# rasd3/TODA

Hardware: NVIDIA B200
Metric: frames/s voxelize+VoxelResBackBone8x fwd+bwd (higher is better)
Workload: dtype bf16

## Files before the change

### include/toda_b200.h

```cpp
#ifndef TODA_B200_H
#define TODA_B200_H

#include <stddef.h>
#include <stdint.h>

#ifdef __cplusplus
extern "C" {
#endif

#define TODA_OK 0
#define TODA_ERR_INVALID (-1)
#define TODA_ERR_CUDA (-2)
#define TODA_ERR_WORKSPACE (-3)
#define TODA_ERR_UNSUPPORTED (-4)

#define TODA_ORDER_FIRST_APPEARANCE 0
#define TODA_ORDER_CANONICAL 1

const char *toda_last_error(void);
int toda_version(void);
long long toda_launch_count(void);
int toda_device_info(int *sm_count_host, int *cc_major_host, int *cc_minor_host);

size_t toda_index_bytes(int batch, int D, int H, int W);
int toda_index_insert(void *index, int batch, int D, int H, int W, const int32_t *coords, int n, void *stream);
int toda_index_insert_strided(void *index_out, int batch, int oD, int oH, int oW, const int32_t *in_coords, int n_in,
                              const int *ksize_host, const int *stride_host, const int *pad_host, void *stream);
int toda_index_build(void *index, int batch, int D, int H, int W, int32_t *out_coords, int cap, int32_t *n_out,
                     void *stream);
int toda_index_rows(const void *index, int batch, int D, int H, int W, const int32_t *coords, int n, int32_t *rows,
                    void *stream);
int toda_index_release(void *index, int batch, int D, int H, int W, const int32_t *coords, int n, void *stream);

#define TODA_SELECT_RANGE_XY 0
#define TODA_SELECT_RECT_XY 1
#define TODA_SELECT_SECTOR 2
#define TODA_SELECT_BOXES 3
size_t toda_points_select_workspace_bytes(int n);
int toda_points_select(const float *points, int n, int stride, int x_col, const int32_t *frame_offsets, int batch, int mode,
                       const double *params_host, int invert, int add_batch_col, float *out, int32_t *out_offsets,
                       void *workspace, size_t workspace_bytes, void *stream);

#define TODA_WORLD_FLIP_X 0
#define TODA_WORLD_FLIP_Y 1
#define TODA_WORLD_ROTATE 2
#define TODA_WORLD_SCALE 3
int toda_points_world_transform(const float *points, int n, int stride, int x_col, const int32_t *frame_offsets, int batch,
                                int n_steps, const int *kinds_host, const float *params_host, float *out, void *stream);

size_t toda_voxelize_workspace_bytes(int64_t n_points, int batch, const int *grid_host, int max_points,
                                     int max_voxels);
int toda_voxelize_hard(const float *points, int64_t n_points, int point_stride, int xyz_col, int feat_col,
                       int num_features, const int32_t *frame_offsets, int batch, const float *range_host,
                       const float *vsize_host, const int *grid_host, int max_points, int max_voxels, int order,
                       float *voxels, int32_t *coords, int32_t *num_points, int32_t *voxel_counts, void *workspace,
                       size_t workspace_bytes, void *stream);

int toda_mean_vfe_fwd(const float *voxels, const void *num_points, int num_is_float, int n_voxels, int max_points,
                      int num_features, float *voxel_features, void *stream);
int toda_mean_vfe_bwd(const float *d_voxel_features, const void *num_points, int num_is_float, int n_voxels,
                      int max_points, int num_features, float *d_voxels, void *stream);

int toda_rulebook_subm(const void *index, int batch, int D, int H, int W, const int32_t *coords, int n,
                       const int *ksize_host, int32_t *nbr, void *stream);
int toda_rulebook_sparse(const void *index_in, int iD, int iH, int iW, const void *index_out, int oD, int oH, int oW,
                         int batch, const int32_t *in_coords, int n_in, const int32_t *out_coords, int n_out,
                         const int *ksize_host, const int *stride_host, const int *pad_host, int32_t *nbr_fwd,
                         int32_t *nbr_bwd, void *stream);

size_t toda_parity_order_workspace_bytes(int n);
int toda_parity_order(const int32_t *coords, int n, const int *stride_host, const int *pad_host, int32_t *order,
                      int32_t *pos_of_row, void *workspace, size_t workspace_bytes, void *stream);

#define TODA_CONV_FP32 0
#define TODA_CONV_BF16 1
#define TODA_CONV_BF16X3 2
int toda_weight_repack(const float *w_param, int kvol, int cin, int cout, int transpose, int mirror_k, float *w_out,
                       void *stream);
size_t toda_spconv_fwd_workspace_bytes(int n_in, int cin, int cout, int kvol, int precision);
int toda_table_tile_masks(const int32_t *nbr, int n_out, int kvol, uint32_t *masks, void *stream);
int toda_spconv_uses_tensor_cores(int cin, int cout, int kvol, int precision);
int toda_spconv_wgrad_uses_tensor_cores(int cin, int cout, int kvol, int precision);
int toda_spconv_fwd(const float *x, const void *x_bf16, int n_in, int cin, const int32_t *nbr, int n_out, int kvol,
                    const float *w, int cout, const float *bias, float *y, const int32_t *out_rows,
                    const uint32_t *tile_masks, double *bn_sums, int precision, void *workspace, size_t workspace_bytes,
                    void *stream);
int toda_tile_plan_capacity(int channels);
int toda_table_tile_plan(const int32_t *nbr, int n_out, int kvol, int ngroups, int cap, uint16_t *lidx, int32_t *rows,
                         int32_t *cnt, void *stream);
int toda_spconv_fwd_plan(const float *x, const void *x_bf16, int n_in, int cin, const int32_t *nbr, int n_out, int kvol,
                         const float *w, int cout, const float *bias, const float *addend, float *y,
                         const int32_t *out_rows, const uint32_t *tile_masks, const uint16_t *plan_lidx,
                         const int32_t *plan_rows, const int32_t *plan_cnt, int plan_groups, int plan_cap, double *bn_sums,
                         const void *w_bf16, int precision, void *workspace, size_t workspace_bytes, void *stream);
int toda_weight_kmajor_bf16(const float *w, int kvol, int cin, int cout, void *w_bf16, void *stream);
size_t toda_spconv_wgrad_workspace_bytes(int n_in, int n_out, int kvol, int cin, int cout, int precision);
int toda_spconv_wgrad(const float *x, const void *x_bf16, int n_in, int cin, const int32_t *nbr, int n_out, int kvol,
                      const uint32_t *tile_masks, const float *dy, const void *dy_bf16, int cout, float *dw_param,
                      void *workspace, size_t workspace_bytes, int precision, void *stream);
int toda_spconv_wgrad_row_splits(const uint32_t *tile_masks, int n_out, int kvol, int cin, int cout, int *groups,
                                 int *splits, int32_t *row_begin, void *stream);

size_t toda_bn_workspace_bytes(int channels);
int toda_bn_local_sums(const float *y, const double *epilogue_sums, int n, int channels, double *sums, double *count,
                       void *workspace, size_t workspace_bytes, void *stream);
int toda_bn_eval_coeffs(const float *gamma, const float *beta, const float *running_mean, const float *running_var,
                        float eps, int channels, float *scale, float *shift, void *stream);
int toda_bn_apply(const float *y, int n, int channels, const float *scale, const float *shift, const float *residual,
                  int relu, float *a, void *a_bf16, void *stream);
int toda_bn_apply_sums(const float *y, int n, int channels, const double *sums, const double *count, const float *gamma,
                       const float *beta, float eps, float momentum, float *running_mean, float *running_var, float *scale,
                       float *shift, float *save_mean, float *save_rstd, const float *residual, int relu, float *a,
                       void *a_bf16, void *stream);
int toda_bn_bwd_reduce(const float *da, const float *a, const float *y, int n, int channels, const float *save_mean,
                       const float *save_rstd, int relu, double *red, float *dgamma, float *dbeta, void *workspace,
                       size_t workspace_bytes, void *stream);
int toda_bn_bwd_finish(const float *da, const float *a, const float *y, int n, int channels, const float *gamma,
                       const float *save_mean, const float *save_rstd, int relu, int training, const double *red,
                       const double *count, float *dy, void *dy_bf16, float *dresidual, float *dbias, void *workspace,
                       size_t workspace_bytes, void *stream);
int toda_bn_bwd(const float *da, const float *a, const float *y, int n, int channels, const float *gamma,
                const float *save_mean, const float *save_rstd, int relu, int training, float *dy, void *dy_bf16,
                float *dresidual, float *dgamma, float *dbeta, float *dbias, void *workspace, size_t workspace_bytes,
                void *stream);
int toda_col_sum(const float *dy, int n, int channels, float *out, void *workspace, size_t workspace_bytes,
                 void *stream);

typedef struct {
    const float *x; const void *x_bf16; int n_in, cin; const int32_t *nbr; int n_out, kvol;
    const float *w; const void *w_bf16 ; int cout; const float *bias ;
    const uint32_t *tile_masks ;
    const uint16_t *plan_lidx ; const int32_t *plan_rows; const int32_t *plan_cnt; int plan_groups, plan_cap;
    int precision; void *conv_ws; size_t conv_ws_bytes;
    const float *gamma; const float *beta; float eps, momentum; float *running_mean; float *running_var; int training;
    const float *residual ; int relu;
    float *y; double *sums; float *stats; float *a; void *a_bf16 ;
    void *bn_ws; size_t bn_ws_bytes;
} toda_layer_fwd_args;
typedef struct {
    const float *da; const float *a_mask; const float *y; int n_out, cout; const float *gamma; const float *mean; const float *rstd;
    int relu, training; float *dy; void *dy_bf16 ; float *dres ; float *dgamma; float *dbeta;
    void *bn_ws; size_t bn_ws_bytes;
    const float *x; const void *x_bf16 ; int n_in, cin, kvol;
    int need_dx; const int32_t *dgrad_nbr; const float *wt; const void *wt_bf16 ;
    const int32_t *dgrad_out_rows ; const uint32_t *dgrad_masks ;
    const uint16_t *dplan_lidx ; const int32_t *dplan_rows; const int32_t *dplan_cnt; int dplan_groups, dplan_cap;
    const float *addend ; float *dx;
    int need_dw; const int32_t *nbr_fwd; const uint32_t *fwd_masks ; float *dw;
    void *wgrad_ws; size_t wgrad_ws_bytes;
    int need_db; float *db;
    int precision; void *conv_ws; size_t conv_ws_bytes;
} toda_layer_bwd_args;
int toda_layer_fwd(const toda_layer_fwd_args *args, void *stream);
int toda_layer_bwd(const toda_layer_bwd_args *args, void *stream);
int toda_layer_fwd_stats(const toda_layer_fwd_args *args, double *local_sums, void *stream);
int toda_layer_fwd_apply(const toda_layer_fwd_args *args, const double *global_sums, void *stream);
int toda_layer_bwd_reduce(const toda_layer_bwd_args *args, double *local_red, void *stream);
int toda_layer_bwd_finish(const toda_layer_bwd_args *args, const double *global_red, const double *global_count, void *stream);

int toda_bev_scatter_fwd(const float *features, const int32_t *coords, int n, int channels, int batch, int D, int H,
                         int W, float *out, void *stream);
int toda_bev_scatter_bwd(const float *d_out, const int32_t *coords, int n, int channels, int batch, int D, int H,
                         int W, float *d_features, void *stream);

int toda_gather_rows(const float *in, const int32_t *rows, int n, int channels, float *out, void *stream);

#ifdef __cplusplus
}
#endif
#endif
```

### toda_b200/_C.py

```python
import ctypes
import os

_HERE = os.path.dirname(os.path.abspath(__file__))
LIB_PATH = os.path.join(_HERE, "lib", "libtoda_b200.so")

c_int, c_i64, c_f32, c_vp, c_sz = ctypes.c_int, ctypes.c_int64, ctypes.c_float, ctypes.c_void_p, ctypes.c_size_t
_IP = ctypes.POINTER(ctypes.c_int)
_FP = ctypes.POINTER(ctypes.c_float)

SIGNATURES = {
    "toda_last_error": (ctypes.c_char_p, []),
    "toda_version": (c_int, []),
    "toda_launch_count": (ctypes.c_longlong, []),
    "toda_device_info": (c_int, [_IP, _IP, _IP]),
    "toda_index_bytes": (c_sz, [c_int] * 4),
    "toda_index_insert": (c_int, [c_vp, c_int, c_int, c_int, c_int, c_vp, c_int, c_vp]),
    "toda_index_insert_strided": (c_int, [c_vp, c_int, c_int, c_int, c_int, c_vp, c_int, _IP, _IP, _IP, c_vp]),
    "toda_index_build": (c_int, [c_vp, c_int, c_int, c_int, c_int, c_vp, c_int, c_vp, c_vp]),
    "toda_index_rows": (c_int, [c_vp, c_int, c_int, c_int, c_int, c_vp, c_int, c_vp, c_vp]),
    "toda_index_release": (c_int, [c_vp, c_int, c_int, c_int, c_int, c_vp, c_int, c_vp]),
    "toda_points_select_workspace_bytes": (c_sz, [c_int]),
    "toda_points_select": (c_int, [c_vp, c_int, c_int, c_int, c_vp, c_int, c_int, ctypes.POINTER(ctypes.c_double), c_int, c_int,
                                   c_vp, c_vp, c_vp, c_sz, c_vp]),
    "toda_points_world_transform": (c_int, [c_vp, c_int, c_int, c_int, c_vp, c_int, c_int, _IP, _FP, c_vp, c_vp]),
    "toda_voxelize_workspace_bytes": (c_sz, [c_i64, c_int, _IP, c_int, c_int]),
    "toda_voxelize_hard": (c_int, [c_vp, c_i64, c_int, c_int, c_int, c_int, c_vp, c_int, _FP, _FP, _IP, c_int, c_int,
                                   c_int, c_vp, c_vp, c_vp, c_vp, c_vp, c_sz, c_vp]),
    "toda_mean_vfe_fwd": (c_int, [c_vp, c_vp, c_int, c_int, c_int, c_int, c_vp, c_vp]),
    "toda_mean_vfe_bwd": (c_int, [c_vp, c_vp, c_int, c_int, c_int, c_int, c_vp, c_vp]),
    "toda_rulebook_subm": (c_int, [c_vp, c_int, c_int, c_int, c_int, c_vp, c_int, _IP, c_vp, c_vp]),
    "toda_rulebook_sparse": (c_int, [c_vp, c_int, c_int, c_int, c_vp, c_int, c_int, c_int, c_int, c_vp, c_int, c_vp,
                                     c_int, _IP, _IP, _IP, c_vp, c_vp, c_vp]),
    "toda_weight_repack": (c_int, [c_vp, c_int, c_int, c_int, c_int, c_int, c_vp, c_vp]),
    "toda_spconv_fwd_workspace_bytes": (c_sz, [c_int] * 5),
    "toda_spconv_uses_tensor_cores": (c_int, [c_int] * 4),
    "toda_spconv_wgrad_uses_tensor_cores": (c_int, [c_int] * 4),
    "toda_parity_order_workspace_bytes": (c_sz, [c_int]),
    "toda_parity_order": (c_int, [c_vp, c_int, _IP, _IP, c_vp, c_vp, c_vp, c_sz, c_vp]),
    "toda_table_tile_masks": (c_int, [c_vp, c_int, c_int, c_vp, c_vp]),
    "toda_spconv_fwd": (c_int, [c_vp, c_vp, c_int, c_int, c_vp, c_int, c_int, c_vp, c_int, c_vp, c_vp, c_vp, c_vp, c_vp, c_int, c_vp,
                                c_sz, c_vp]),
    "toda_tile_plan_capacity": (c_int, [c_int]),
    "toda_table_tile_plan": (c_int, [c_vp, c_int, c_int, c_int, c_int, c_vp, c_vp, c_vp, c_vp]),
    "toda_spconv_fwd_plan": (c_int, [c_vp, c_vp, c_int, c_int, c_vp, c_int, c_int, c_vp, c_int, c_vp, c_vp, c_vp, c_vp, c_vp, c_vp,
                                     c_vp, c_vp, c_int, c_int, c_vp, c_vp, c_int, c_vp, c_sz, c_vp]),
    "toda_weight_kmajor_bf16": (c_int, [c_vp, c_int, c_int, c_int, c_vp, c_vp]),
    "toda_layer_fwd": (c_int, [c_vp, c_vp]),
    "toda_layer_bwd": (c_int, [c_vp, c_vp]),
    "toda_layer_fwd_stats": (c_int, [c_vp, c_vp, c_vp]),
    "toda_layer_fwd_apply": (c_int, [c_vp, c_vp, c_vp]),
    "toda_layer_bwd_reduce": (c_int, [c_vp, c_vp, c_vp]),
    "toda_layer_bwd_finish": (c_int, [c_vp, c_vp, c_vp, c_vp]),
    "toda_spconv_wgrad_workspace_bytes": (c_sz, [c_int] * 6),
    "toda_spconv_wgrad": (c_int, [c_vp, c_vp, c_int, c_int, c_vp, c_int, c_int, c_vp, c_vp, c_vp, c_int, c_vp, c_vp, c_sz, c_int,
                                  c_vp]),
    "toda_spconv_wgrad_row_splits": (c_int, [c_vp, c_int, c_int, c_int, c_int, _IP, _IP, c_vp, c_vp]),
    "toda_bn_workspace_bytes": (c_sz, [c_int]),
    "toda_bn_local_sums": (c_int, [c_vp, c_vp, c_int, c_int, c_vp, c_vp, c_vp, c_sz, c_vp]),
    "toda_bn_eval_coeffs": (c_int, [c_vp, c_vp, c_vp, c_vp, c_f32, c_int, c_vp, c_vp, c_vp]),
    "toda_bn_apply": (c_int, [c_vp, c_int, c_int, c_vp, c_vp, c_vp, c_int, c_vp, c_vp, c_vp]),
    "toda_bn_apply_sums": (c_int, [c_vp, c_int, c_int, c_vp, c_vp, c_vp, c_vp, c_f32, c_f32, c_vp, c_vp, c_vp, c_vp, c_vp, c_vp,
                                   c_vp, c_int, c_vp, c_vp, c_vp]),
    "toda_bn_bwd": (c_int, [c_vp, c_vp, c_vp, c_int, c_int, c_vp, c_vp, c_vp, c_int, c_int, c_vp, c_vp, c_vp, c_vp, c_vp,
                            c_vp, c_vp, c_sz, c_vp]),
    "toda_bn_bwd_reduce": (c_int, [c_vp, c_vp, c_vp, c_int, c_int, c_vp, c_vp, c_int, c_vp, c_vp, c_vp, c_vp, c_sz, c_vp]),
    "toda_bn_bwd_finish": (c_int, [c_vp, c_vp, c_vp, c_int, c_int, c_vp, c_vp, c_vp, c_int, c_int, c_vp, c_vp, c_vp, c_vp, c_vp,
                                   c_vp, c_vp, c_sz, c_vp]),
    "toda_col_sum": (c_int, [c_vp, c_int, c_int, c_vp, c_vp, c_sz, c_vp]),
    "toda_bev_scatter_fwd": (c_int, [c_vp, c_vp, c_int, c_int, c_int, c_int, c_int, c_int, c_vp, c_vp]),
    "toda_bev_scatter_bwd": (c_int, [c_vp, c_vp, c_int, c_int, c_int, c_int, c_int, c_int, c_vp, c_vp]),
    "toda_gather_rows": (c_int, [c_vp, c_vp, c_int, c_int, c_vp, c_vp]),
}



class LayerFwdArgs(ctypes.Structure):
    _fields_ = [("x", c_vp), ("x_bf16", c_vp), ("n_in", c_int), ("cin", c_int), ("nbr", c_vp), ("n_out", c_int), ("kvol", c_int),
                ("w", c_vp), ("w_bf16", c_vp), ("cout", c_int), ("bias", c_vp), ("tile_masks", c_vp),
                ("plan_lidx", c_vp), ("plan_rows", c_vp), ("plan_cnt", c_vp), ("plan_groups", c_int), ("plan_cap", c_int),
                ("precision", c_int), ("conv_ws", c_vp), ("conv_ws_bytes", c_sz),
                ("gamma", c_vp), ("beta", c_vp), ("eps", c_f32), ("momentum", c_f32), ("running_mean", c_vp), ("running_var", c_vp),
                ("training", c_int), ("residual", c_vp), ("relu", c_int),
                ("y", c_vp), ("sums", c_vp), ("stats", c_vp), ("a", c_vp), ("a_bf16", c_vp), ("bn_ws", c_vp), ("bn_ws_bytes", c_sz)]


class LayerBwdArgs(ctypes.Structure):
    _fields_ = [("da", c_vp), ("a_mask", c_vp), ("y", c_vp), ("n_out", c_int), ("cout", c_int), ("gamma", c_vp), ("mean", c_vp),
                ("rstd", c_vp), ("relu", c_int), ("training", c_int), ("dy", c_vp), ("dy_bf16", c_vp), ("dres", c_vp), ("dgamma", c_vp),
                ("dbeta", c_vp), ("bn_ws", c_vp), ("bn_ws_bytes", c_sz),
                ("x", c_vp), ("x_bf16", c_vp), ("n_in", c_int), ("cin", c_int), ("kvol", c_int),
                ("need_dx", c_int), ("dgrad_nbr", c_vp), ("wt", c_vp), ("wt_bf16", c_vp), ("dgrad_out_rows", c_vp), ("dgrad_masks", c_vp),
                ("dplan_lidx", c_vp), ("dplan_rows", c_vp), ("dplan_cnt", c_vp), ("dplan_groups", c_int), ("dplan_cap", c_int),
                ("addend", c_vp), ("dx", c_vp),
                ("need_dw", c_int), ("nbr_fwd", c_vp), ("fwd_masks", c_vp), ("dw", c_vp), ("wgrad_ws", c_vp), ("wgrad_ws_bytes", c_sz),
                ("need_db", c_int), ("db", c_vp),
                ("precision", c_int), ("conv_ws", c_vp), ("conv_ws_bytes", c_sz)]


_lib = None


def lib():
    global _lib
    if _lib is None:
        if not os.path.exists(LIB_PATH):
            raise RuntimeError(
                f"{LIB_PATH} is missing: build it with `python -c 'import __graft_entry__ as g; g.build()'` "
                "(nvcc, sm_100a).  toda_b200 has no CPU fallback.")
        L = ctypes.CDLL(LIB_PATH)
        for name, (res, args) in SIGNATURES.items():
            fn = getattr(L, name)
            fn.restype = res
            fn.argtypes = args
        _lib = L
    return _lib


def check(rc, what=""):
    if rc != 0:
        msg = lib().toda_last_error().decode("utf-8", "replace")
        raise RuntimeError(f"libtoda_b200 {what} failed (code {rc}): {msg}")


def ints(vals):
    return (ctypes.c_int * len(vals))(*[int(v) for v in vals])


def doubles(vals):
    return (ctypes.c_double * len(vals))(*[float(v) for v in vals])


def floats(vals):
    return (ctypes.c_float * len(vals))(*[float(v) for v in vals])
```

### toda_b200/csrc/bn.cu

```cuda
#include <cuda_bf16.h>

#include "common.cuh"

namespace {

constexpr int kThreads = 256;
constexpr int kPartials = 2 * kNumSMs;
constexpr int kApplyPartials = 2048 / kThreads * kNumSMs;

template <int MODE>
__global__ void __launch_bounds__(kThreads) col_reduce_vec_kernel(const float *__restrict__ p0, const float *__restrict__ p1,
                                                                  const float *__restrict__ p2, int n, int c,
                                                                  const float *__restrict__ mean, const float *__restrict__ rstd,
                                                                  int relu, double *__restrict__ partial) {
    __shared__ double s0[kThreads * 4], s1[kThreads * 4];
    const int tpr = c >> 2;
    const int rpi = kThreads / tpr;
    const int tx = threadIdx.x % tpr, ty = threadIdx.x / tpr;
    double a0[4] = {0, 0, 0, 0}, a1[4] = {0, 0, 0, 0};
    float4 m4 = make_float4(0, 0, 0, 0), r4 = make_float4(0, 0, 0, 0);
    if (MODE == 1) { m4 = __ldg((const float4 *)mean + tx); r4 = __ldg((const float4 *)rstd + tx); }
    const long long stride = (long long)gridDim.x * rpi;
    const bool active = ty < rpi;
    constexpr int U = 4;
    for (long long r = (long long)blockIdx.x * rpi + ty; active && r < n; r += U * stride) {
        float4 v0[U], v1[U], v2[U];
        bool ok[U];
#pragma unroll
        for (int u = 0; u < U; ++u) {
            long long rr = r + u * stride;
            ok[u] = rr < n;
            size_t e = ok[u] ? (size_t)rr * tpr + tx : 0;
            v0[u] = __ldg((const float4 *)p0 + e);
            if (MODE == 1) { v1[u] = __ldg((const float4 *)p1 + e); v2[u] = __ldg((const float4 *)p2 + e); }
        }
#pragma unroll
        for (int u = 0; u < U; ++u) {
            if (!ok[u]) continue;
            float x[4] = {v0[u].x, v0[u].y, v0[u].z, v0[u].w};
            if (MODE == 0) {
#pragma unroll
                for (int q = 0; q < 4; ++q) { a0[q] += x[q]; a1[q] += (double)x[q] * x[q]; }
            } else if (MODE == 1) {
                float av[4] = {v1[u].x, v1[u].y, v1[u].z, v1[u].w}, yv[4] = {v2[u].x, v2[u].y, v2[u].z, v2[u].w};
                float mm[4] = {m4.x, m4.y, m4.z, m4.w}, rs[4] = {r4.x, r4.y, r4.z, r4.w};
#pragma unroll
                for (int q = 0; q < 4; ++q) {
                    float g = (relu && !(av[q] > 0.f)) ? 0.f : x[q];
                    float xh = (yv[q] - mm[q]) * rs[q];
                    a0[q] += g; a1[q] += (double)g * xh;
                }
            } else {
#pragma unroll
                for (int q = 0; q < 4; ++q) a0[q] += x[q];
            }
        }
    }
#pragma unroll
    for (int q = 0; q < 4; ++q) { s0[threadIdx.x * 4 + q] = a0[q]; s1[threadIdx.x * 4 + q] = a1[q]; }
    __syncthreads();
    if ((int)threadIdx.x < c) {
        int ch = threadIdx.x, txx = ch >> 2, q = ch & 3;
        double t0 = 0.0, t1 = 0.0;
        for (int j = 0; j < rpi; ++j) { t0 += s0[(j * tpr + txx) * 4 + q]; t1 += s1[(j * tpr + txx) * 4 + q]; }
        partial[((size_t)blockIdx.x * 2 + 0) * c + ch] = t0;
        partial[((size_t)blockIdx.x * 2 + 1) * c + ch] = t1;
    }
}

template <int MODE>
__global__ void __launch_bounds__(kThreads) col_reduce_kernel(const float *__restrict__ p0, const float *__restrict__ p1,
                                                              const float *__restrict__ p2, int n, int c,
                                                              const float *__restrict__ mean, const float *__restrict__ rstd,
                                                              int relu, double *__restrict__ partial) {
    __shared__ double s0[kThreads], s1[kThreads];
    const int cpad = c <= 16 ? 16 : (c <= 32 ? 32 : (c <= 64 ? 64 : (c <= 128 ? 128 : 256)));
    const int rows_per_iter = kThreads / cpad;
    const int tx = threadIdx.x % cpad, ty = threadIdx.x / cpad;
    double a0 = 0.0, a1 = 0.0;
    float m = 0.f, rs = 0.f;
    if (MODE == 1 && tx < c) { m = mean[tx]; rs = rstd[tx]; }
    for (long long r = (long long)blockIdx.x * rows_per_iter + ty; r < n; r += (long long)gridDim.x * rows_per_iter) {
        if (tx < c) {
            size_t e = (size_t)r * c + tx;
            if (MODE == 0) {
                float v = __ldg(p0 + e);
                a0 += v; a1 += (double)v * v;
            } else if (MODE == 1) {
                float g = __ldg(p0 + e);
                if (relu && !(__ldg(p1 + e) > 0.f)) g = 0.f;
                float xh = (__ldg(p2 + e) - m) * rs;
                a0 += g; a1 += (double)g * xh;
            } else {
                a0 += __ldg(p0 + e);
            }
        }
    }
    s0[threadIdx.x] = a0; s1[threadIdx.x] = a1;
    __syncthreads();
    if (threadIdx.x < cpad && threadIdx.x < c) {
        double t0 = 0.0, t1 = 0.0;
        for (int j = 0; j < rows_per_iter; ++j) { t0 += s0[j * cpad + threadIdx.x]; t1 += s1[j * cpad + threadIdx.x]; }
        partial[((size_t)blockIdx.x * 2 + 0) * c + threadIdx.x] = t0;
        partial[((size_t)blockIdx.x * 2 + 1) * c + threadIdx.x] = t1;
    }
}

static bool vec_channels(int c) { return c % 4 == 0 && kThreads % (c / 4) == 0; }

template <int MODE>
static void launch_col_reduce(const float *p0, const float *p1, const float *p2, int n, int c, const float *mean,
                              const float *rstd, int relu, double *partial, cudaStream_t st) {
    if (vec_channels(c))
        col_reduce_vec_kernel<MODE><<<kPartials, kThreads, 0, st>>>(p0, p1, p2, n, c, mean, rstd, relu, partial);
    else
        col_reduce_kernel<MODE><<<kPartials, kThreads, 0, st>>>(p0, p1, p2, n, c, mean, rstd, relu, partial);
}

template <int MAX_BLOCKS = kPartials, int ROWS = 2>
__device__ __forceinline__ void warp_sum_partials(const double *__restrict__ partial, int nblocks, int c, int ch, double &s,
                                                  double &ss) {
    const int lane = threadIdx.x & 31;
    constexpr int kPerLane = (MAX_BLOCKS + 31) / 32;
    double va[kPerLane], vb[kPerLane];
#pragma unroll
    for (int i = 0; i < kPerLane; ++i) {
        const int j = lane + 32 * i;
        const bool ok = j < nblocks;
        va[i] = ok ? partial[((size_t)j * ROWS) * c + ch] : 0.0;
        vb[i] = ok && ROWS == 2 ? partial[((size_t)j * ROWS + 1) * c + ch] : 0.0;
    }
    double a = 0.0, b = 0.0;
#pragma unroll
    for (int i = 0; i < kPerLane; ++i) { a += va[i]; b += vb[i]; }
#pragma unroll
    for (int o = 16; o > 0; o >>= 1) { a += __shfl_xor_sync(0xffffffffu, a, o); b += __shfl_xor_sync(0xffffffffu, b, o); }
    s = a; ss = b;
}

__device__ __forceinline__ void bn_coeffs(double s, double ss, int n, float g, float bt, float eps, float &scale, float &shift,
                                          float &meanf, float &rstd, double &var) {
    const double mean = n > 0 ? s / n : 0.0;
    var = n > 0 ? ss / n - mean * mean : 0.0;
    if (var < 0.0) var = 0.0;
    rstd = (float)(1.0 / sqrt(var + (double)eps));
    meanf = (float)mean;
    scale = __fmul_rn(g, rstd);
    shift = __fsub_rn(bt, __fmul_rn(__fmul_rn(meanf, g), rstd));
}

__device__ __forceinline__ void bn_update_running(float *running_mean, float *running_var, int ch, float momentum, float meanf,
                                                  double var, int n) {
    if (running_mean) running_mean[ch] = __fadd_rn(__fmul_rn(1.f - momentum, running_mean[ch]), __fmul_rn(momentum, meanf));
    if (running_var) {
        const double unbiased = n > 1 ? var * n / (n - 1) : var;
        running_var[ch] = __fadd_rn(__fmul_rn(1.f - momentum, running_var[ch]), __fmul_rn(momentum, (float)unbiased));
    }
}

__global__ void bn_local_sums_kernel(const double *partial, int nblocks, const double *src, int n, int c, double *out,
                                     double *count) {
    if (count && blockIdx.x == 0 && threadIdx.x == 0) *count = (double)n;
    int ch = (blockIdx.x * blockDim.x + threadIdx.x) >> 5;
    if (ch >= c) return;
    double s = 0.0, ss = 0.0;
    if (partial) warp_sum_partials(partial, nblocks, c, ch, s, ss);
    else if (src) { s = src[ch]; ss = src[c + ch]; }
    if ((threadIdx.x & 31) != 0) return;
    out[ch] = s;
    out[c + ch] = ss;
}

__global__ void bn_eval_coeffs_kernel(const float *gamma, const float *beta, const float *rm, const float *rv, float eps,
                                      int c, float *scale, float *shift) {
    int ch = blockIdx.x * blockDim.x + threadIdx.x;
    if (ch >= c) return;
    float rstd = 1.0f / sqrtf(rv[ch] + eps);
    float g = gamma ? gamma[ch] : 1.f, bt = beta ? beta[ch] : 0.f;
    scale[ch] = g * rstd;
    shift[ch] = bt - rm[ch] * g * rstd;
}

__device__ __forceinline__ void store_bf16x4(__nv_bfloat16 *__restrict__ dst, long long e, float4 o) {
    __nv_bfloat162 lo = __floats2bfloat162_rn(o.x, o.y), hi = __floats2bfloat162_rn(o.z, o.w);
    uint2 pk;
    pk.x = *(uint32_t *)&lo;
    pk.y = *(uint32_t *)&hi;
    ((uint2 *)dst)[e] = pk;
}

struct BnCoeffs {
    const double *sums; const double *count; int n;
    const float *gamma, *beta; float eps, momentum;
    float *running_mean, *running_var, *scale, *shift, *save_mean, *save_rstd;
};

template <bool VEC>
__global__ void __launch_bounds__(kThreads) bn_apply_kernel(const float *__restrict__ y, long long total, int c, BnCoeffs k,
                                                            const float *__restrict__ residual, int relu, float *__restrict__ a,
                                                            __nv_bfloat16 *__restrict__ a_bf16) {
    extern __shared__ __align__(16) float s_coef[];
    float *s_sc = s_coef, *s_sh = s_coef + c;
    const int n = k.count ? (int)*k.count : k.n;
    for (int ch = threadIdx.x; ch < c; ch += blockDim.x) {
        if (!k.sums) {
            s_sc[ch] = k.scale[ch];
            s_sh[ch] = k.shift[ch];
            continue;
        }
        float meanf, rstd;
        double var;
        bn_coeffs(k.sums[ch], k.sums[c + ch], n, k.gamma ? k.gamma[ch] : 1.f, k.beta ? k.beta[ch] : 0.f, k.eps, s_sc[ch], s_sh[ch],
                  meanf, rstd, var);
        if (blockIdx.x == 0) {
            k.scale[ch] = s_sc[ch];
            k.shift[ch] = s_sh[ch];
            if (k.save_mean) k.save_mean[ch] = meanf;
            if (k.save_rstd) k.save_rstd[ch] = rstd;
            if (n > 0) bn_update_running(k.running_mean, k.running_var, ch, k.momentum, meanf, var, n);
        }
    }
    __syncthreads();
    const long long stride = (long long)gridDim.x * blockDim.x;
    long long e = blockIdx.x * (long long)blockDim.x + threadIdx.x;
    if (VEC) {
        const long long tv = total >> 2;
        const int ch = (int)((e << 2) % c);
        const float4 sc = *(const float4 *)(s_sc + ch), sh = *(const float4 *)(s_sh + ch);
        for (; e < tv; e += stride) {
            const float4 v = __ldg((const float4 *)y + e);
            float4 o = make_float4(fmaf(v.x, sc.x, sh.x), fmaf(v.y, sc.y, sh.y), fmaf(v.z, sc.z, sh.z), fmaf(v.w, sc.w, sh.w));
            if (residual) {
                const float4 r = __ldg((const float4 *)residual + e);
                o.x += r.x; o.y += r.y; o.z += r.z; o.w += r.w;
            }
            if (relu) { o.x = fmaxf(o.x, 0.f); o.y = fmaxf(o.y, 0.f); o.z = fmaxf(o.z, 0.f); o.w = fmaxf(o.w, 0.f); }
            ((float4 *)a)[e] = o;
            if (a_bf16) store_bf16x4(a_bf16, e, o);
        }
    } else {
        for (; e < total; e += stride) {
            const int ch = (int)(e % c);
            float o = fmaf(__ldg(y + e), s_sc[ch], s_sh[ch]);
            if (residual) o += __ldg(residual + e);
            if (relu) o = fmaxf(o, 0.f);
            a[e] = o;
            if (a_bf16) a_bf16[e] = __float2bfloat16_rn(o);
        }
    }
}

__global__ void bn_bwd_finalize_kernel(const double *__restrict__ partial, int nblocks, int c, float *dgamma, float *dbeta,
                                       double *sums) {
    int ch = (blockIdx.x * blockDim.x + threadIdx.x) >> 5;
    if (ch >= c) return;
    double s, sx;
    warp_sum_partials(partial, nblocks, c, ch, s, sx);
    if ((threadIdx.x & 31) != 0) return;
    if (dbeta) dbeta[ch] = (float)s;
    if (dgamma) dgamma[ch] = (float)sx;
    sums[ch] = s;
    sums[c + ch] = sx;
}

template <bool VEC>
__global__ void __launch_bounds__(kThreads, 5) bn_bwd_apply_kernel(const float *__restrict__ da, const float *__restrict__ a,
                                                                const float *__restrict__ y, long long total, int c, int n,
                                                                const double *__restrict__ count, const float *__restrict__ gamma,
                                                                const float *__restrict__ mean, const float *__restrict__ rstd,
                                                                const double *__restrict__ sums, int relu, int training,
                                                                float *__restrict__ dy, float *__restrict__ dres,
                                                                __nv_bfloat16 *__restrict__ dy_bf16, double *__restrict__ db_partial) {
    extern __shared__ double s_db[];
    double db[4] = {0.0, 0.0, 0.0, 0.0};
    if (count) n = (int)*count;
    auto sum = [&](int i) -> float { return (float)sums[i]; };
    const float inv_n = n > 0 ? 1.0f / (float)n : 0.f;
    const long long threads = (long long)gridDim.x * blockDim.x;
    const long long stride = VEC ? threads : threads / c * c;
    long long e = blockIdx.x * (long long)blockDim.x + threadIdx.x;
    if (VEC) {
        const long long tv = total >> 2;
        const int ch = (int)((e << 2) % c);
        float A[4], B[4], C[4];
#pragma unroll
        for (int q = 0; q < 4; ++q) {
            float gm = gamma ? gamma[ch + q] : 1.f, rs = rstd[ch + q];
            A[q] = gm * rs;
            B[q] = training ? -gm * rs * rs * sum(c + ch + q) * inv_n : 0.f;
            C[q] = training ? -A[q] * sum(ch + q) * inv_n - B[q] * mean[ch + q] : 0.f;
        }
        for (; e < tv; e += stride) {
            float4 g4 = __ldg((const float4 *)da + e);
            float4 y4 = training ? __ldg((const float4 *)y + e) : make_float4(0.f, 0.f, 0.f, 0.f);
            if (relu) {
                float4 a4 = __ldg((const float4 *)a + e);
                g4.x = a4.x > 0.f ? g4.x : 0.f; g4.y = a4.y > 0.f ? g4.y : 0.f;
                g4.z = a4.z > 0.f ? g4.z : 0.f; g4.w = a4.w > 0.f ? g4.w : 0.f;
            }
            if (dres) ((float4 *)dres)[e] = g4;
            float4 o;
            o.x = fmaf(A[0], g4.x, fmaf(B[0], y4.x, C[0]));
            o.y = fmaf(A[1], g4.y, fmaf(B[1], y4.y, C[1]));
            o.z = fmaf(A[2], g4.z, fmaf(B[2], y4.z, C[2]));
            o.w = fmaf(A[3], g4.w, fmaf(B[3], y4.w, C[3]));
            if (dy) ((float4 *)dy)[e] = o;
            if (dy_bf16) store_bf16x4(dy_bf16, e, o);
            if (db_partial) { db[0] += o.x; db[1] += o.y; db[2] += o.z; db[3] += o.w; }
        }
    } else {
        for (e = e < stride ? e : total; e < total; e += stride) {
            int ch = (int)(e % c);
            float g = __ldg(da + e);
            if (relu && !(__ldg(a + e) > 0.f)) g = 0.f;
            if (dres) dres[e] = g;
            float gm = gamma ? gamma[ch] : 1.f;
            float rs = rstd[ch];
            float o;
            if (training) {
                float xh = (__ldg(y + e) - mean[ch]) * rs;
                o = gm * rs * (g - sum(ch) * inv_n - xh * sum(c + ch) * inv_n);
            } else {
                o = gm * rs * g;
            }
            if (dy) dy[e] = o;
            if (dy_bf16) dy_bf16[e] = __float2bfloat16_rn(o);
            if (db_partial) db[0] += o;
        }
    }
    if (!db_partial) return;
    constexpr int kSlots = VEC ? 4 : 1;
#pragma unroll
    for (int q = 0; q < kSlots; ++q) s_db[threadIdx.x * kSlots + q] = db[q];
    __syncthreads();
    if ((int)threadIdx.x < c) {
        const int units = VEC ? c / 4 : c;
        const int u = VEC ? (int)threadIdx.x >> 2 : (int)threadIdx.x, q = VEC ? (int)threadIdx.x & 3 : 0;
        double t = 0.0;
        for (int j = u; j < kThreads; j += units) t += s_db[j * kSlots + q];
        const int ch = VEC ? (int)threadIdx.x : (int)(((long long)blockIdx.x * kThreads + threadIdx.x) % c);
        db_partial[(size_t)blockIdx.x * c + ch] = t;
    }
}

template <int MAX_BLOCKS, int ROWS>
__global__ void col_sum_finalize_kernel(const double *__restrict__ partial, int nblocks, int c, float *out) {
    int ch = (blockIdx.x * blockDim.x + threadIdx.x) >> 5;
    if (ch >= c) return;
    double s, unused;
    warp_sum_partials<MAX_BLOCKS, ROWS>(partial, nblocks, c, ch, s, unused);
    if ((threadIdx.x & 31) == 0) out[ch] = (float)s;
}

size_t partials_bytes(int c) {
    return (size_t)(2 * kPartials > kApplyPartials ? 2 * kPartials : kApplyPartials) * c * sizeof(double);
}
size_t bn_ws_bytes(int c) { return align_up(partials_bytes(c) + 2 * c * sizeof(double), 256); }

template <auto Kernel> int resident_grid(int64_t items) {
    static const int64_t cap = [] {
        int per_sm = 0;
        if (cudaOccupancyMaxActiveBlocksPerMultiprocessor(&per_sm, Kernel, kThreads, 0) != cudaSuccess || per_sm < 1) per_sm = 4;
        return (int64_t)per_sm * kNumSMs;
    }();
    const int64_t need = (items + kThreads - 1) / kThreads;
    return (int)(need < 1 ? 1 : (need < cap ? need : cap));
}

int launch_bn_apply(const float *y, int n, int c, const BnCoeffs &k, const float *residual, int relu, float *a, void *a_bf16,
                    cudaStream_t st) {
    const long long total = (long long)n * c;
    const size_t smem = 2 * (size_t)c * sizeof(float);
    if (vec_channels(c))
        bn_apply_kernel<true><<<resident_grid<bn_apply_kernel<true>>(total / 4), kThreads, smem, st>>>(
            y, total, c, k, residual, relu, a, (__nv_bfloat16 *)a_bf16);
    else
        bn_apply_kernel<false><<<resident_grid<bn_apply_kernel<false>>(total), kThreads, smem, st>>>(
            y, total, c, k, residual, relu, a, (__nv_bfloat16 *)a_bf16);
    TODA_LAUNCH_OK();
    return TODA_OK;
}

}

extern "C" size_t toda_bn_workspace_bytes(int channels) { return channels > 0 ? bn_ws_bytes(channels) : 0; }

double *bn_workspace_red(void *workspace, int c) { return (double *)((char *)workspace + partials_bytes(c)); }

extern "C" int toda_bn_local_sums(const float *y, const double *epilogue_sums, int n, int c, double *sums, double *count,
                                  void *workspace, size_t workspace_bytes, void *stream) {
    TODA_CHECK_ARG(n >= 0 && c > 0 && c <= 256 && sums, "bn_local_sums: bad args n=%d c=%d", n, c);
    if (n > 0 && epilogue_sums == sums && !count) return TODA_OK;
    cudaStream_t st = (cudaStream_t)stream;
    const double *partial = nullptr;
    if (n > 0 && !epilogue_sums) {
        TODA_CHECK_ARG(y && workspace, "bn_local_sums: null pointer");
        if (workspace_bytes < bn_ws_bytes(c)) { toda_set_error("bn_local_sums: workspace too small"); return TODA_ERR_WORKSPACE; }
        launch_col_reduce<0>(y, nullptr, nullptr, n, c, nullptr, nullptr, 0, (double *)workspace, st);
        TODA_LAUNCH_OK();
        partial = (const double *)workspace;
    }
    bn_local_sums_kernel<<<ceil_div(c * 32, 128), 128, 0, st>>>(partial, kPartials, n > 0 ? epilogue_sums : nullptr, n, c, sums,
                                                              count);
    TODA_LAUNCH_OK();
    return TODA_OK;
}

extern "C" int toda_bn_eval_coeffs(const float *gamma, const float *beta, const float *running_mean, const float *running_var,
                                   float eps, int c, float *scale, float *shift, void *stream) {
    TODA_CHECK_ARG(c > 0 && running_mean && running_var && scale && shift, "bn_eval_coeffs: bad args");
    bn_eval_coeffs_kernel<<<ceil_div(c, 128), 128, 0, (cudaStream_t)stream>>>(gamma, beta, running_mean, running_var, eps, c,
                                                                             scale, shift);
    TODA_LAUNCH_OK();
    return TODA_OK;
}

extern "C" int toda_bn_apply(const float *y, int n, int c, const float *scale, const float *shift, const float *residual,
                             int relu, float *a, void *a_bf16, void *stream) {
    TODA_CHECK_ARG(n >= 0 && c > 0, "bn_apply: bad sizes");
    if (n == 0) return TODA_OK;
    TODA_CHECK_ARG(y && scale && shift && a, "bn_apply: null pointer");
    BnCoeffs k{};
    k.scale = (float *)scale;
    k.shift = (float *)shift;
    return launch_bn_apply(y, n, c, k, residual, relu, a, a_bf16, (cudaStream_t)stream);
}

extern "C" int toda_bn_apply_sums(const float *y, int n, int c, const double *sums, const double *count, const float *gamma,
                                  const float *beta, float eps, float momentum, float *running_mean, float *running_var,
                                  float *scale, float *shift, float *save_mean, float *save_rstd, const float *residual, int relu,
                                  float *a, void *a_bf16, void *stream) {
    TODA_CHECK_ARG(n >= 0 && c > 0 && sums && scale && shift, "bn_apply_sums: bad args");
    TODA_CHECK_ARG(n == 0 || (y && a), "bn_apply_sums: null pointer");
    const BnCoeffs k{sums, count, n, gamma, beta, eps, momentum, running_mean, running_var, scale, shift, save_mean, save_rstd};
    return launch_bn_apply(y, n, c, k, residual, relu, a, a_bf16, (cudaStream_t)stream);
}

extern "C" int toda_bn_bwd_reduce(const float *da, const float *a, const float *y, int n, int c, const float *save_mean,
                                  const float *save_rstd, int relu, double *local_red, float *dgamma, float *dbeta, void *workspace,
                                  size_t workspace_bytes, void *stream) {
    TODA_CHECK_ARG(n >= 0 && c > 0 && c <= 256, "bn_bwd_reduce: unsupported sizes n=%d c=%d", n, c);
    TODA_CHECK_ARG(save_mean && save_rstd && workspace && local_red && (n == 0 || (da && y)) && (!relu || a || n == 0),
                   "bn_bwd_reduce: null pointer");
    if (workspace_bytes < bn_ws_bytes(c)) { toda_set_error("bn_bwd_reduce: workspace too small"); return TODA_ERR_WORKSPACE; }
    cudaStream_t st = (cudaStream_t)stream;
    double *partial = (double *)workspace;
    launch_col_reduce<1>(da, a, y, n, c, save_mean, save_rstd, relu, partial, st);
    TODA_LAUNCH_OK();
    bn_bwd_finalize_kernel<<<ceil_div(c * 32, 128), 128, 0, st>>>(partial, kPartials, c, dgamma, dbeta, local_red);
    TODA_LAUNCH_OK();
    return TODA_OK;
}

extern "C" int toda_bn_bwd_finish(const float *da, const float *a, const float *y, int n, int c, const float *gamma,
                                  const float *save_mean, const float *save_rstd, int relu, int training, const double *red,
                                  const double *count, float *dy, void *dy_bf16, float *dresidual, float *dbias, void *workspace,
                                  size_t workspace_bytes, void *stream) {
    TODA_CHECK_ARG(n >= 0 && c > 0 && c <= 256, "bn_bwd_finish: unsupported sizes n=%d c=%d", n, c);
    TODA_CHECK_ARG(save_mean && save_rstd && (red || !training) && (n == 0 || (da && y && (dy || dy_bf16))) &&
                   (!relu || a || n == 0) && (!dbias || workspace), "bn_bwd_finish: null pointer");
    cudaStream_t st = (cudaStream_t)stream;
    if (dbias && workspace_bytes < bn_ws_bytes(c)) { toda_set_error("bn_bwd_finish: workspace too small"); return TODA_ERR_WORKSPACE; }
    if (n == 0) {
        if (dbias) TODA_CUDA_OK(cudaMemsetAsync(dbias, 0, sizeof(float) * c, st));
        return TODA_OK;
    }
    const long long total = (long long)n * c;
    double *db_partial = dbias ? (double *)workspace : nullptr;
    const size_t smem = dbias ? kThreads * 4 * sizeof(double) : 0;
    int grid;
    if (vec_channels(c)) {
        grid = resident_grid<bn_bwd_apply_kernel<true>>(total / 4);
        grid = grid < kApplyPartials ? grid : kApplyPartials;
        bn_bwd_apply_kernel<true><<<grid, kThreads, smem, st>>>(da, a, y, total, c, n, count, gamma, save_mean, save_rstd, red, relu,
                                                               training, dy, dresidual, (__nv_bfloat16 *)dy_bf16, db_partial);
    } else {
        grid = resident_grid<bn_bwd_apply_kernel<false>>(total);
        grid = grid < kApplyPartials ? grid : kApplyPartials;
        bn_bwd_apply_kernel<false><<<grid, kThreads, smem, st>>>(da, a, y, total, c, n, count, gamma, save_mean, save_rstd, red,
                                                                relu, training, dy, dresidual, (__nv_bfloat16 *)dy_bf16, db_partial);
    }
    TODA_LAUNCH_OK();
    if (dbias) {
        col_sum_finalize_kernel<kApplyPartials, 1><<<ceil_div(c * 32, 128), 128, 0, st>>>(db_partial, grid, c, dbias);
        TODA_LAUNCH_OK();
    }
    return TODA_OK;
}

extern "C" int toda_bn_bwd(const float *da, const float *a, const float *y, int n, int c, const float *gamma,
                           const float *save_mean, const float *save_rstd, int relu, int training, float *dy, void *dy_bf16,
                           float *dresidual, float *dgamma, float *dbeta, float *dbias, void *workspace, size_t workspace_bytes,
                           void *stream) {
    TODA_CHECK_ARG(workspace, "bn_bwd: null workspace");
    double *red = bn_workspace_red(workspace, c);
    int rc = toda_bn_bwd_reduce(da, a, y, n, c, save_mean, save_rstd, relu, red, dgamma, dbeta, workspace, workspace_bytes, stream);
    if (rc) return rc;
    return toda_bn_bwd_finish(da, a, y, n, c, gamma, save_mean, save_rstd, relu, training, red, nullptr, dy, dy_bf16, dresidual,
                              dbias, workspace, workspace_bytes, stream);
}

extern "C" int toda_col_sum(const float *dy, int n, int c, float *out, void *workspace, size_t workspace_bytes, void *stream) {
    TODA_CHECK_ARG(n >= 0 && c > 0 && c <= 256 && out && workspace, "col_sum: bad args");
    if (workspace_bytes < bn_ws_bytes(c)) { toda_set_error("col_sum: workspace too small"); return TODA_ERR_WORKSPACE; }
    cudaStream_t st = (cudaStream_t)stream;
    double *partial = (double *)workspace;
    launch_col_reduce<2>(dy, nullptr, nullptr, n, c, nullptr, nullptr, 0, partial, st);
    TODA_LAUNCH_OK();
    col_sum_finalize_kernel<kPartials, 2><<<ceil_div(c * 32, 128), 128, 0, st>>>(partial, kPartials, c, out);
    TODA_LAUNCH_OK();
    return TODA_OK;
}
```

### toda_b200/csrc/common.cuh

```cuda
#pragma once
#include <cuda_runtime.h>
#include <stdint.h>
#include <stdio.h>

#include "../../include/toda_b200.h"

#if defined(__CUDA_ARCH__) && (__CUDA_ARCH__ < 1000)
#error "libtoda_b200 targets sm_100a (B200) only"
#endif

void toda_set_error(const char *fmt, ...);

#define TODA_CHECK_ARG(cond, ...)            \
    do {                                      \
        if (!(cond)) {                        \
            toda_set_error(__VA_ARGS__);      \
            return TODA_ERR_INVALID;          \
        }                                     \
    } while (0)

#define TODA_CUDA_OK(expr)                                                                   \
    do {                                                                                      \
        cudaError_t _e = (expr);                                                              \
        if (_e != cudaSuccess) {                                                              \
            toda_set_error("%s:%d CUDA error: %s", __FILE__, __LINE__, cudaGetErrorString(_e)); \
            return TODA_ERR_CUDA;                                                             \
        }                                                                                     \
    } while (0)

extern long long g_toda_launches;
#define TODA_LAUNCH_OK() do { ++g_toda_launches; TODA_CUDA_OK(cudaGetLastError()); } while (0)

constexpr int kNumSMs = 148;

static inline int ceil_div(int64_t a, int64_t b) { return (int)((a + b - 1) / b); }
static inline size_t align_up(size_t x, size_t a) { return (x + a - 1) / a * a; }

static inline int wave_grid(int64_t n, int block, int waves = 8) {
    int64_t need = (n + block - 1) / block;
    if (need <= 0) need = 1;
    int64_t rounded = (need + kNumSMs - 1) / kNumSMs * kNumSMs;
    int64_t cap = (int64_t)kNumSMs * waves;
    return (int)(rounded < cap ? rounded : cap);
}

double *bn_workspace_red(void *workspace, int c);

struct GridIndex {
    unsigned long long *bits0;
    int *rank0;
    unsigned long long *bits1;
    int *pref1;
    int *tile_sums;
    long long frame_stride;
    long long words0;
    int words1;
    int batch, D, H, W;
};

static inline long long index_frame_stride(int D, int H, int W) {
    long long c = (long long)D * H * W;
    return (c + 4095) / 4096 * 4096;
}

static inline size_t index_layout(GridIndex *g, void *base, int batch, int D, int H, int W) {
    long long fs = index_frame_stride(D, H, W);
    long long cells = fs * batch;
    long long words0 = cells / 64;
    long long words1 = words0 / 64;
    size_t off = 0;
    char *p = (char *)base;
    size_t o_bits0 = off; off = align_up(off + (size_t)words0 * 8, 256);
    size_t o_bits1 = off; off = align_up(off + (size_t)words1 * 8, 256);
    size_t zero_bytes = off;
    size_t o_rank0 = off; off = align_up(off + (size_t)words0 * 4, 256);
    size_t o_pref1 = off; off = align_up(off + (size_t)(words1 + 1) * 4, 256);
    size_t o_tiles = off; off = align_up(off + (size_t)(words1 / 1024 + 2) * 4, 256);
    if (g) {
        g->bits0 = (unsigned long long *)(p + o_bits0);
        g->bits1 = (unsigned long long *)(p + o_bits1);
        g->rank0 = (int *)(p + o_rank0);
        g->pref1 = (int *)(p + o_pref1);
        g->tile_sums = (int *)(p + o_tiles);
        g->frame_stride = fs;
        g->words0 = words0;
        g->words1 = (int)words1;
        g->batch = batch; g->D = D; g->H = H; g->W = W;
    }
    (void)zero_bytes;
    return off;
}

__device__ __forceinline__ long long index_cell(const GridIndex &g, int b, int z, int y, int x) {
    return (long long)b * g.frame_stride + ((long long)z * g.H + y) * g.W + x;
}

__device__ __forceinline__ int index_lookup(const GridIndex &g, long long cell) {
    unsigned long long w = __ldg(g.bits0 + (cell >> 6));
    unsigned bit = (unsigned)(cell & 63);
    if (!((w >> bit) & 1ull)) return -1;
    return __ldg(g.rank0 + (cell >> 6)) + __popcll(w & ((1ull << bit) - 1ull));
}

__device__ __forceinline__ void index_mark(const GridIndex &g, long long cell) {
    unsigned long long *wp = g.bits0 + (cell >> 6);
    unsigned long long m = 1ull << (cell & 63);
    if (*wp & m) return;
    unsigned long long old = atomicOr(wp, m);
    if (old == 0ull) {
        long long w = cell >> 6;
        atomicOr(g.bits1 + (w >> 6), 1ull << (w & 63));
    }
}

int index_build_ranks(const GridIndex &g, int32_t *out_coords, int cap, uint32_t *out_cells, int32_t *n_out,
                      cudaStream_t st);
int scan_exclusive_i32(const int *in, int *out, int n, int *tile_sums, int *total_out, cudaStream_t st);
```

### toda_b200/csrc/layer.cu

```cuda
#include "common.cuh"

static int layer_conv(const toda_layer_fwd_args *p, double *bn_sums, void *stream) {
    return toda_spconv_fwd_plan(p->x, p->x_bf16, p->n_in, p->cin, p->nbr, p->n_out, p->kvol, p->w, p->cout, p->bias, nullptr, p->y,
                                nullptr, p->tile_masks, p->plan_lidx, p->plan_rows, p->plan_cnt, p->plan_groups, p->plan_cap,
                                bn_sums, p->w_bf16, p->precision, p->conv_ws, p->conv_ws_bytes, stream);
}

static int layer_fwd_stats(const toda_layer_fwd_args *p, double *sums, double *count, void *stream) {
    const int c = p->cout, n = p->n_out;
    const bool tc = n > 0 && toda_spconv_uses_tensor_cores(p->cin, c, p->kvol, p->precision);
    int rc = layer_conv(p, tc ? sums : nullptr, stream);
    if (rc) return rc;
    return toda_bn_local_sums(p->y, tc ? sums : nullptr, n, c, sums, count, p->bn_ws, p->bn_ws_bytes, stream);
}

static int layer_fwd_apply(const toda_layer_fwd_args *p, const double *sums, const double *count, void *stream) {
    const int c = p->cout;
    float *scale = p->stats, *shift = p->stats + c, *mean = p->stats + 2 * c, *rstd = p->stats + 3 * c;
    return toda_bn_apply_sums(p->y, p->n_out, c, sums, count, p->gamma, p->beta, p->eps, p->momentum, p->running_mean,
                              p->running_var, scale, shift, mean, rstd, p->residual, p->relu, p->a, p->a_bf16, stream);
}

extern "C" int toda_layer_fwd(const toda_layer_fwd_args *p, void *stream) {
    TODA_CHECK_ARG(p, "layer_fwd: null args");
    const int c = p->cout, n = p->n_out;
    TODA_CHECK_ARG(c > 0 && n >= 0 && p->stats && (n == 0 || (p->y && p->a)) && (!p->training || p->sums),
                   "layer_fwd: bad sizes / null outputs");
    if (n == 0) return layer_conv(p, nullptr, stream);
    int rc;
    if (p->training) {
        rc = layer_fwd_stats(p, p->sums, nullptr, stream);
        return rc ? rc : layer_fwd_apply(p, p->sums, nullptr, stream);
    }
    float *scale = p->stats, *shift = p->stats + c;
    if ((rc = layer_conv(p, nullptr, stream))) return rc;
    if ((rc = toda_bn_eval_coeffs(p->gamma, p->beta, p->running_mean, p->running_var, p->eps, c, scale, shift, stream))) return rc;
    return toda_bn_apply(p->y, n, c, scale, shift, p->residual, p->relu, p->a, p->a_bf16, stream);
}

static int layer_bwd_empty(const toda_layer_bwd_args *p, bool bn_grads, cudaStream_t st) {
    const int c = p->cout;
    if (bn_grads && p->dgamma) TODA_CUDA_OK(cudaMemsetAsync(p->dgamma, 0, sizeof(float) * c, st));
    if (bn_grads && p->dbeta) TODA_CUDA_OK(cudaMemsetAsync(p->dbeta, 0, sizeof(float) * c, st));
    if (p->need_db && p->db) TODA_CUDA_OK(cudaMemsetAsync(p->db, 0, sizeof(float) * c, st));
    if (p->need_dw && p->dw) TODA_CUDA_OK(cudaMemsetAsync(p->dw, 0, sizeof(float) * (size_t)p->kvol * p->cin * c, st));
    if (p->need_dx && p->dx && p->n_in > 0) {
        if (p->addend) TODA_CUDA_OK(cudaMemcpyAsync(p->dx, p->addend, sizeof(float) * (size_t)p->n_in * p->cin, cudaMemcpyDeviceToDevice, st));
        else TODA_CUDA_OK(cudaMemsetAsync(p->dx, 0, sizeof(float) * (size_t)p->n_in * p->cin, st));
    }
    return TODA_OK;
}

static bool layer_bwd_reads_dy_f32(const toda_layer_bwd_args *p) {
    const int c = p->cout;
    return !p->dy_bf16 || p->precision != TODA_CONV_BF16 ||
           (p->need_dx && !toda_spconv_uses_tensor_cores(c, p->cin, p->kvol, p->precision)) ||
           (p->need_dw && !toda_spconv_wgrad_uses_tensor_cores(p->cin, c, p->kvol, p->precision));
}

static int layer_bwd_conv(const toda_layer_bwd_args *p, void *stream) {
    const int c = p->cout, n = p->n_out;
    int rc;
    if (p->need_dx) {
        rc = toda_spconv_fwd_plan(p->dy, p->dy_bf16, n, c, p->dgrad_nbr, p->n_in, p->kvol, p->wt, p->cin, nullptr, p->addend, p->dx,
                                  p->dgrad_out_rows, p->dgrad_masks, p->dplan_lidx, p->dplan_rows, p->dplan_cnt, p->dplan_groups,
                                  p->dplan_cap, nullptr, p->wt_bf16, p->precision, p->conv_ws, p->conv_ws_bytes, stream);
        if (rc) return rc;
    }
    if (p->need_dw) {
        rc = toda_spconv_wgrad(p->x, p->x_bf16, p->n_in, p->cin, p->nbr_fwd, n, p->kvol, p->fwd_masks, p->dy, p->dy_bf16, c, p->dw,
                               p->wgrad_ws, p->wgrad_ws_bytes, p->precision, stream);
        if (rc) return rc;
    }
    return TODA_OK;
}

static int layer_bwd_reduce(const toda_layer_bwd_args *p, double *red, void *stream) {
    return toda_bn_bwd_reduce(p->da, p->a_mask, p->y, p->n_out, p->cout, p->mean, p->rstd, p->relu, red, p->dgamma, p->dbeta,
                              p->bn_ws, p->bn_ws_bytes, stream);
}

static int layer_bwd_finish(const toda_layer_bwd_args *p, const double *red, const double *count, void *stream) {
    const int c = p->cout, n = p->n_out;
    if (n == 0) return layer_bwd_empty(p, false, (cudaStream_t)stream);
    int rc = toda_bn_bwd_finish(p->da, p->a_mask, p->y, n, c, p->gamma, p->mean, p->rstd, p->relu, p->training, red, count,
                                layer_bwd_reads_dy_f32(p) ? p->dy : nullptr, p->dy_bf16, p->dres, p->need_db ? p->db : nullptr,
                                p->bn_ws, p->bn_ws_bytes, stream);
    return rc ? rc : layer_bwd_conv(p, stream);
}

extern "C" int toda_layer_bwd(const toda_layer_bwd_args *p, void *stream) {
    TODA_CHECK_ARG(p, "layer_bwd: null args");
    TODA_CHECK_ARG(p->cout > 0 && p->n_out >= 0, "layer_bwd: bad sizes");
    if (p->n_out == 0) return layer_bwd_empty(p, true, (cudaStream_t)stream);
    TODA_CHECK_ARG(p->bn_ws, "layer_bwd: null workspace");
    double *red = bn_workspace_red(p->bn_ws, p->cout);
    int rc = layer_bwd_reduce(p, red, stream);
    return rc ? rc : layer_bwd_finish(p, red, nullptr, stream);
}


extern "C" int toda_layer_fwd_stats(const toda_layer_fwd_args *p, double *local_sums, void *stream) {
    TODA_CHECK_ARG(p && local_sums, "layer_fwd_stats: null args");
    const int c = p->cout, n = p->n_out;
    TODA_CHECK_ARG(c > 0 && n >= 0 && p->training && (n == 0 || p->y), "layer_fwd_stats: bad sizes / not training / null y");
    return layer_fwd_stats(p, local_sums, local_sums + 2 * c, stream);
}

extern "C" int toda_layer_fwd_apply(const toda_layer_fwd_args *p, const double *global_sums, void *stream) {
    TODA_CHECK_ARG(p && global_sums, "layer_fwd_apply: null args");
    const int c = p->cout, n = p->n_out;
    TODA_CHECK_ARG(c > 0 && n >= 0 && p->training && p->stats && (n == 0 || (p->y && p->a)),
                   "layer_fwd_apply: bad sizes / not training / null outputs");
    return layer_fwd_apply(p, global_sums, global_sums + 2 * c, stream);
}

extern "C" int toda_layer_bwd_reduce(const toda_layer_bwd_args *p, double *local_red, void *stream) {
    TODA_CHECK_ARG(p && local_red, "layer_bwd_reduce: null args");
    TODA_CHECK_ARG(p->cout > 0 && p->n_out >= 0 && p->training, "layer_bwd_reduce: bad sizes / not training");
    return layer_bwd_reduce(p, local_red, stream);
}

extern "C" int toda_layer_bwd_finish(const toda_layer_bwd_args *p, const double *global_red, const double *global_count,
                                     void *stream) {
    TODA_CHECK_ARG(p && global_red && global_count, "layer_bwd_finish: null args");
    TODA_CHECK_ARG(p->cout > 0 && p->n_out >= 0 && p->training, "layer_bwd_finish: bad sizes / not training");
    return layer_bwd_finish(p, global_red, global_count, stream);
}
```

### toda_b200/ops.py

```python
import ctypes
import weakref
from dataclasses import dataclass
from typing import List, Optional

import numpy as np
import torch
import torch.distributed as dist

from . import _C

ORDER_FIRST_APPEARANCE = 0
ORDER_CANONICAL = 1
CONV_FP32 = 0
CONV_BF16 = 1
CONV_BF16X3 = 2
_TC_PRECISIONS = (CONV_BF16, CONV_BF16X3)

_launch_base = 0


def launches():
    return int(_C.lib().toda_launch_count()) - _launch_base


def reset_launches():
    global _launch_base
    _launch_base = int(_C.lib().toda_launch_count())



_prof = None


def profile_begin():
    global _prof
    _prof = []


def profile_end():
    global _prof
    rec, _prof = _prof, None
    torch.cuda.synchronize()
    return [dict(name=n, ms=a.elapsed_time(b), **m) for (n, m, a, b) in rec]


class _Timed:
    def __init__(self, name, meta):
        self.name, self.meta = name, meta

    def __enter__(self):
        self.a = torch.cuda.Event(enable_timing=True)
        self.a.record()
        return self

    def __exit__(self, *exc):
        b = torch.cuda.Event(enable_timing=True)
        b.record()
        _prof.append((self.name, self.meta, self.a, b))
        return False


class _NoTimer:
    def __enter__(self):
        return self

    def __exit__(self, *exc):
        return False


_NO_TIMER = _NoTimer()


def _timed(name, **meta):
    return _Timed(name, meta) if _prof is not None else _NO_TIMER


_raw_stream = torch._C._cuda_getCurrentRawStream


def _stream_id(device=None):
    return _raw_stream(torch.cuda.current_device() if device is None or device.index is None else device.index)


def _stream():
    return ctypes.c_void_p(_raw_stream(torch.cuda.current_device()))


def _p(t: Optional[torch.Tensor]):
    return ctypes.c_void_p(t.data_ptr()) if t is not None else None


def _need(t, dtype, name):
    if not t.is_cuda:
        raise RuntimeError(f"{name} must be a CUDA tensor (toda_b200 has no CPU path)")
    if t.dtype != dtype:
        raise TypeError(f"{name} must be {dtype}, got {t.dtype}")
    if not t.is_contiguous():
        raise ValueError(f"{name} must be contiguous")
    return t


_workspaces = {}


def _workspace(tag, nbytes, device, zero=False):
    key = (tag, device.index, _stream_id(device))
    buf = _workspaces.get(key)
    if buf is None or buf.numel() < nbytes:
        buf = (torch.zeros if zero else torch.empty)(int(nbytes * 1.25) + 256, dtype=torch.uint8, device=device)
        _workspaces[key] = buf
    return buf


SELECT_RANGE_XY, SELECT_RECT_XY, SELECT_SECTOR, SELECT_BOXES = 0, 1, 2, 3
SELECT_MAX_BOXES = 96


def points_select(points, frame_offsets, mode, params, invert=False, add_batch_col=False, x_col=0, trim=True):
    points = _need(points, torch.float32, "points")
    assert points.dim() == 2
    n, stride = points.shape
    dev = points.device
    batch = 0
    if frame_offsets is not None:
        frame_offsets = _need(frame_offsets, torch.int32, "frame_offsets")
        batch = frame_offsets.numel() - 1
    L = _C.lib()
    ws = _workspace("select", L.toda_points_select_workspace_bytes(n), dev)
    out = torch.empty((n, stride + (1 if add_batch_col else 0)), dtype=torch.float32, device=dev)
    out_offsets = torch.empty((batch + 1,), dtype=torch.int32, device=dev)
    p = list(params) + [0.0] * (4 - len(params))
    with _timed("points_select", n=n, stride=stride, mode=int(mode)):
        _C.check(L.toda_points_select(_p(points), n, stride, int(x_col), _p(frame_offsets), batch, int(mode), _C.doubles(p),
                                      int(bool(invert)), int(bool(add_batch_col)), _p(out), _p(out_offsets), _p(ws),
                                      ws.numel(), _stream()), "toda_points_select")
    if trim:
        return out[:int(out_offsets[-1].item())], out_offsets
    return out, out_offsets


WORLD_FLIP_X, WORLD_FLIP_Y, WORLD_ROTATE, WORLD_SCALE = 0, 1, 2, 3
WORLD_MAX_STEPS = 4
WORLD_MAX_BATCH = 64


def points_world_transform(points, frame_offsets, steps, x_col=0):
    points = _need(points, torch.float32, "points")
    if points.dim() != 2:
        raise ValueError("points must be (N, stride)")
    n, stride = points.shape
    if not (0 <= x_col and x_col + 2 < stride <= 63):
        raise ValueError(f"points_world_transform: x, y, z at columns {x_col}..{x_col + 2} do not fit stride {stride} (<= 63)")
    batch = 1
    if frame_offsets is not None:
        frame_offsets = _need(frame_offsets, torch.int32, "frame_offsets")
        batch = frame_offsets.numel() - 1
        if not 1 <= batch <= WORLD_MAX_BATCH:
            raise ValueError(f"points_world_transform: batch {batch} outside [1, {WORLD_MAX_BATCH}]")
    if len(steps) > WORLD_MAX_STEPS:
        raise ValueError(f"points_world_transform: {len(steps)} steps (at most {WORLD_MAX_STEPS})")
    kinds, params = [], np.zeros((len(steps), batch, 2), np.float32)
    for s, (kind, values) in enumerate(steps):
        if kind not in (WORLD_FLIP_X, WORLD_FLIP_Y, WORLD_ROTATE, WORLD_SCALE):
            raise ValueError(f"points_world_transform: unknown step kind {kind!r}")
        v = np.asarray(values, dtype=np.float32).reshape(batch, -1)
        if v.shape[1] != (2 if kind == WORLD_ROTATE else 1):
            raise ValueError(f"points_world_transform: step {s} needs {2 if kind == WORLD_ROTATE else 1} value(s) per frame for "
                             f"{batch} frame(s), got {np.shape(values)}")
        kinds.append(int(kind))
        params[s, :, :v.shape[1]] = v
    out = torch.empty_like(points)
    with _timed("points_world_transform", n=n, stride=stride, steps=len(steps)):
        _C.check(_C.lib().toda_points_world_transform(_p(points), n, stride, int(x_col), _p(frame_offsets), batch, len(kinds),
                                                      _C.ints(kinds or [0]), _C.floats(params.reshape(-1).tolist() or [0.0]),
                                                      _p(out), _stream()), "toda_points_world_transform")
    return out


def gather_point_rows(points, rows):
    points = _need(points, torch.float32, "points")
    rows = _need(rows, torch.int32, "rows")
    n, c = rows.shape[0], points.shape[1]
    out = torch.empty((n, c), dtype=torch.float32, device=points.device)
    _C.check(_C.lib().toda_gather_rows(_p(points), _p(rows), n, c, _p(out), _stream()), "toda_gather_rows")
    return out


def grid_size_xyz(pc_range, voxel_size):
    r = np.asarray(pc_range, dtype=np.float64)
    return np.round((r[3:6] - r[0:3]) / np.asarray(voxel_size, dtype=np.float64)).astype(np.int64)


def voxelize(points, frame_offsets, pc_range, voxel_size, max_points, max_voxels, num_features=None, xyz_col=0,
             feat_col=0, order=ORDER_FIRST_APPEARANCE, grid=None, trim=True):
    points = _need(points, torch.float32, "points")
    assert points.dim() == 2
    n, stride = points.shape
    dev = points.device
    if not torch.is_tensor(frame_offsets):
        frame_offsets = torch.tensor(list(frame_offsets), dtype=torch.int32, device=dev)
    frame_offsets = _need(frame_offsets, torch.int32, "frame_offsets")
    batch = frame_offsets.numel() - 1
    f = int(num_features) if num_features is not None else stride - feat_col
    grid = grid_size_xyz(pc_range, voxel_size) if grid is None else np.asarray(grid)
    grid_c = _C.ints(grid)
    L = _C.lib()
    ws_bytes = L.toda_voxelize_workspace_bytes(n, batch, grid_c, max_points, max_voxels)
    if ws_bytes == 0:
        raise RuntimeError("toda_voxelize_workspace_bytes rejected the arguments")
    ws = _workspace("vox", ws_bytes, dev)
    cap = batch * max_voxels
    voxels = torch.empty((cap, max_points, f), dtype=torch.float32, device=dev)
    coords = torch.empty((cap, 4), dtype=torch.int32, device=dev)
    num = torch.empty((cap,), dtype=torch.int32, device=dev)
    counts = torch.empty((batch + 1,), dtype=torch.int32, device=dev)
    with _timed("voxelize", n_points=n, batch=batch, K=max_points, F=f):
        rc = L.toda_voxelize_hard(_p(points), n, stride, xyz_col, feat_col, f, _p(frame_offsets), batch,
                                  _C.floats(np.asarray(pc_range, dtype=np.float32)),
                                  _C.floats(np.asarray(voxel_size, dtype=np.float32)), grid_c, max_points, max_voxels,
                                  order, _p(voxels), _p(coords), _p(num), _p(counts), _p(ws), ws.numel(), _stream())
    _C.check(rc, "toda_voxelize_hard")
    if trim:
        v = int(counts[batch].item())
        return voxels[:v], coords[:v], num[:v], counts
    return voxels, coords, num, counts


class _MeanVFE(torch.autograd.Function):
    @staticmethod
    def forward(ctx, voxels, num_points):
        voxels = _need(voxels, torch.float32, "voxels")
        v, k, f = voxels.shape
        is_float = num_points.dtype == torch.float32
        if not is_float:
            num_points = _need(num_points, torch.int32, "voxel_num_points")
        num_points = num_points.contiguous()
        out = torch.empty((v, f), dtype=torch.float32, device=voxels.device)
        with _timed("mean_vfe_fwd", V=v, K=k, F=f):
            _C.check(_C.lib().toda_mean_vfe_fwd(_p(voxels), _p(num_points), int(is_float), v, k, f, _p(out), _stream()),
                     "toda_mean_vfe_fwd")
        ctx.save_for_backward(num_points)
        ctx.shape = (v, k, f, is_float)
        return out

    @staticmethod
    def backward(ctx, dout):
        (num_points,) = ctx.saved_tensors
        v, k, f, is_float = ctx.shape
        dout = dout.contiguous()
        dv = torch.empty((v, k, f), dtype=torch.float32, device=dout.device)
        _C.check(_C.lib().toda_mean_vfe_bwd(_p(dout), _p(num_points), int(is_float), v, k, f, _p(dv), _stream()),
                 "toda_mean_vfe_bwd")
        return dv, None


def mean_vfe(voxels, num_points):
    return _MeanVFE.apply(voxels, num_points)


_index_occupant = {}


class OccupancyIndex:

    def __init__(self, batch, shape, device, tag):
        self.batch = int(batch)
        self.shape = [int(s) for s in shape]
        d, h, w = self.shape
        nbytes = _C.lib().toda_index_bytes(self.batch, d, h, w)
        if nbytes == 0:
            raise RuntimeError(f"bad index dims {batch} {shape}")
        self.key = (("index", tag, self.batch, d, h, w), device.index, _stream_id(device))
        self.buf = _workspace(self.key[0], nbytes, device, zero=True)
        self.coords = None
        self.frame_counts = None
        self.n = 0
        self._marked = False

    def _dims(self):
        return (self.batch, *self.shape)

    def _acquire(self):
        prev = _index_occupant.get(self.key)
        if prev is not None and prev is not self and prev.buf.data_ptr() == self.buf.data_ptr():
            prev._unmark()
        _index_occupant[self.key] = self

    def _unmark(self):
        if self.coords is not None and self.n > 0:
            _C.check(_C.lib().toda_index_release(_p(self.buf), *self._dims(), _p(self.coords), self.n, _stream()),
                     "toda_index_release")
        if _index_occupant.get(self.key) is self:
            del _index_occupant[self.key]

    def insert(self, coords):
        self._acquire()
        coords = _need(coords, torch.int32, "coords")
        _C.check(_C.lib().toda_index_insert(_p(self.buf), *self._dims(), _p(coords), coords.shape[0], _stream()),
                 "toda_index_insert")

    def insert_strided(self, in_coords, ksize, stride, padding):
        self._acquire()
        in_coords = _need(in_coords, torch.int32, "in_coords")
        _C.check(_C.lib().toda_index_insert_strided(_p(self.buf), *self._dims(), _p(in_coords), in_coords.shape[0],
                                                    _C.ints(ksize), _C.ints(stride), _C.ints(padding), _stream()),
                 "toda_index_insert_strided")

    def build(self, cap, known_n=None):
        dev = self.buf.device
        coords = torch.empty((max(cap, 1), 4), dtype=torch.int32, device=dev)
        n_out = torch.empty((self.batch + 1,), dtype=torch.int32, device=dev)
        with _timed("index_build", cells=self.batch * self.shape[0] * self.shape[1] * self.shape[2]):
            _C.check(_C.lib().toda_index_build(_p(self.buf), *self._dims(), _p(coords), cap, _p(n_out), _stream()),
                     "toda_index_build")
        self.n = int(n_out[0].item()) if known_n is None else int(known_n)
        self.coords = coords[:self.n]
        self.frame_counts = n_out
        return self.coords

    def ensure_live(self):
        if _index_occupant.get(self.key) is self:
            return
        if self.coords is None:
            raise RuntimeError("occupancy index was released")
        coords, n = self.coords, self.n
        self.insert(coords)
        self.build(n, known_n=n)

    def rows(self, coords):
        self.ensure_live()
        coords = _need(coords, torch.int32, "coords")
        rows = torch.empty((coords.shape[0],), dtype=torch.int32, device=coords.device)
        _C.check(_C.lib().toda_index_rows(_p(self.buf), *self._dims(), _p(coords), coords.shape[0], _p(rows), _stream()),
                 "toda_index_rows")
        return rows

    def release(self):
        if _index_occupant.get(self.key) is self:
            self._unmark()
        self.coords = None
        self.n = 0


@dataclass
class Rulebook:
    subm: bool
    ksize: List[int]
    stride: List[int]
    padding: List[int]
    in_shape: List[int]
    out_shape: List[int]
    n_in: int
    n_out: int
    out_coords: torch.Tensor
    nbr_fwd: torch.Tensor
    nbr_bwd: Optional[torch.Tensor]
    dgrad_order: Optional[torch.Tensor] = None
    nbr_bwd_sorted: Optional[torch.Tensor] = None
    dgrad_tile_masks: Optional[torch.Tensor] = None
    tile_masks: Optional[torch.Tensor] = None
    plan: Optional["TilePlan"] = None
    dgrad_plan: Optional["TilePlan"] = None

    @property
    def kvol(self):
        return self.ksize[0] * self.ksize[1] * self.ksize[2]


@dataclass
class TilePlan:
    lidx: torch.Tensor
    rows: torch.Tensor
    cnt: torch.Tensor
    ngroups: int
    cap: int

    def tensors(self):
        return [self.lidx, self.rows, self.cnt]


def table_tile_plan(nbr, ksize, channels):
    kvol, n = nbr.shape
    ngroups = int(ksize[0])
    if n == 0 or kvol > 27 or ngroups > 3 or kvol % ngroups or kvol // ngroups > 9 or not channels:
        return None
    L = _C.lib()
    cap = L.toda_tile_plan_capacity(int(channels))
    if cap <= 0:
        return None
    tiles = (n + 127) // 128
    dev = nbr.device
    lidx = torch.empty((tiles, kvol, 128), dtype=torch.int16, device=dev)
    rows = torch.empty((tiles, ngroups, cap), dtype=torch.int32, device=dev)
    cnt = torch.empty((tiles, ngroups), dtype=torch.int32, device=dev)
    with _timed("tile_plan", n=n, kvol=kvol):
        _C.check(L.toda_table_tile_plan(_p(nbr), n, kvol, ngroups, cap, _p(lidx), _p(rows), _p(cnt), _stream()),
                 "toda_table_tile_plan")
    return TilePlan(lidx, rows, cnt, ngroups, cap)


def conv_out_size(in_size, k, s, p):
    return (in_size + 2 * p - (k - 1) - 1) // s + 1


def rulebook_subm(index: OccupancyIndex, ksize, channels=None):
    index.ensure_live()
    n = index.n
    kvol = ksize[0] * ksize[1] * ksize[2]
    nbr = torch.empty((kvol, n), dtype=torch.int32, device=index.buf.device)
    with _timed("rulebook_subm", n=n, kvol=kvol):
        _C.check(_C.lib().toda_rulebook_subm(_p(index.buf), index.batch, *index.shape, _p(index.coords), n, _C.ints(ksize),
                                             _p(nbr), _stream()), "toda_rulebook_subm")
    rb = Rulebook(True, list(ksize), [1, 1, 1], [k // 2 for k in ksize], index.shape, index.shape, n, n, index.coords,
                  nbr, None)
    rb.tile_masks = table_tile_masks(nbr) if (n > 0 and kvol <= 32) else None
    rb.plan = table_tile_plan(nbr, ksize, channels) if _TILE_PLANS else None
    return rb


def rulebook_sparse(index_in: OccupancyIndex, ksize, stride, padding, tag, cin=None, cout=None):
    index_in.ensure_live()
    out_shape = [conv_out_size(index_in.shape[a], ksize[a], stride[a], padding[a]) for a in range(3)]
    index_out = OccupancyIndex(index_in.batch, out_shape, index_in.buf.device, tag)
    if index_out.buf.data_ptr() == index_in.buf.data_ptr():
        index_out = OccupancyIndex(index_in.batch, out_shape, index_in.buf.device, (tag, "alt"))
    assert index_out.buf.data_ptr() != index_in.buf.data_ptr()
    index_out.insert_strided(index_in.coords, ksize, stride, padding)
    per_in = 1
    for a in range(3):
        per_in *= min(ksize[a], (ksize[a] + stride[a] - 1) // stride[a])
    cells = index_in.batch * out_shape[0] * out_shape[1] * out_shape[2]
    cap = int(min(index_in.n * per_in, cells))
    out_coords = index_out.build(cap)
    n_in, n_out = index_in.n, index_out.n
    kvol = ksize[0] * ksize[1] * ksize[2]
    dev = index_in.buf.device
    nbr_fwd = torch.empty((kvol, n_out), dtype=torch.int32, device=dev)
    nbr_bwd = torch.empty((kvol, n_in), dtype=torch.int32, device=dev)
    with _timed("rulebook_sparse", n_in=n_in, n_out=n_out, kvol=kvol):
        _C.check(_C.lib().toda_rulebook_sparse(_p(index_in.buf), *index_in.shape, _p(index_out.buf), *out_shape,
                                               index_in.batch, _p(index_in.coords), n_in, _p(out_coords), n_out,
                                               _C.ints(ksize), _C.ints(stride), _C.ints(padding), _p(nbr_fwd), _p(nbr_bwd),
                                               _stream()), "toda_rulebook_sparse")
    rb = Rulebook(False, list(ksize), list(stride), list(padding), index_in.shape, out_shape, n_in, n_out, out_coords,
                  nbr_fwd, nbr_bwd)
    rb.tile_masks = table_tile_masks(nbr_fwd) if (n_out > 0 and kvol <= 32) else None
    rb.dgrad_order, rb.nbr_bwd_sorted = (_dgrad_parity_order(index_in.coords, nbr_bwd, stride, padding) if kvol <= 32
                                         else (None, None))
    if rb.dgrad_order is not None:
        rb.dgrad_tile_masks = table_tile_masks(rb.nbr_bwd_sorted)
    if _TILE_PLANS:
        rb.plan = table_tile_plan(nbr_fwd, ksize, cin)
        rb.dgrad_plan = table_tile_plan(rb.nbr_bwd_sorted if rb.dgrad_order is not None else nbr_bwd, ksize, cout)
    return rb, index_out


import os as _os
_TILE_PLANS = _os.environ.get("TODA_TILE_PLANS", "0") == "1"


def set_tile_plans(on):
    global _TILE_PLANS
    _TILE_PLANS = bool(on)


def tile_plans_enabled():
    return _TILE_PLANS


def table_tile_masks(nbr):
    kvol, n = nbr.shape
    masks = torch.empty(((n + 127) // 128,), dtype=torch.int32, device=nbr.device)
    _C.check(_C.lib().toda_table_tile_masks(_p(nbr), n, kvol, _p(masks), _stream()), "toda_table_tile_masks")
    return masks


def _dgrad_parity_order(in_coords, nbr_bwd, stride, padding):
    if all(s == 1 for s in stride) or in_coords.shape[0] == 0:
        return None, None
    if stride[0] * stride[1] * stride[2] > 8:
        return None, None
    n = in_coords.shape[0]
    L = _C.lib()
    ws = _workspace("parity", L.toda_parity_order_workspace_bytes(n), in_coords.device)
    order = torch.empty((n,), dtype=torch.int32, device=in_coords.device)
    _C.check(L.toda_parity_order(_p(in_coords), n, _C.ints(stride), _C.ints(padding), _p(order), None, _p(ws), ws.numel(),
                                 _stream()), "toda_parity_order")
    return order, nbr_bwd.index_select(1, order).contiguous()


_repack_cache = {}


def invalidate_weight_cache():
    _repack_cache.clear()


def _repack(weight, transpose, mirror, want_bf16=False):
    key = (id(weight), bool(transpose), bool(mirror))
    hit = _repack_cache.get(key)
    if hit is not None and hit[2]() is weight and hit[0] == weight._version and hit[3] == weight.data_ptr():
        out = hit[1]
    else:
        cout, kvol, cin = weight.shape[0], weight.shape[1] * weight.shape[2] * weight.shape[3], weight.shape[4]
        out = torch.empty((kvol, cout, cin) if transpose else (kvol, cin, cout), dtype=torch.float32, device=weight.device)
        _C.check(_C.lib().toda_weight_repack(_p(weight), kvol, cin, cout, int(transpose), int(mirror), _p(out), _stream()),
                 "toda_weight_repack")
        if len(_repack_cache) > 512:
            _repack_cache.clear()
        hit = [weight._version, out, weakref.ref(weight), weight.data_ptr(), None]
        _repack_cache[key] = hit
    if not want_bf16:
        return out
    if hit[4] is None:
        kvol, ci, co = out.shape
        wb = torch.empty((co, kvol * max(ci, 16)), dtype=torch.bfloat16, device=out.device)
        _C.check(_C.lib().toda_weight_kmajor_bf16(_p(out), kvol, ci, co, _p(wb), _stream()), "toda_weight_kmajor_bf16")
        hit[4] = wb
    return out, hit[4]


def _bf16_shadow_of(t):
    tag = getattr(t, "_toda_bf16", None)
    if tag is not None and tag[1] == t._version and tag[0].shape == t.shape:
        return tag[0]
    return None


def _conv_call(x, xb, cin, nbr, n_out, kvol, w, cout, bias, precision, what="conv_fwd", rb=None, bn_sums=None, y=None,
               out_rows=None, tile_masks=None, plan=None, addend=None, w_bf16=None):
    if y is None:
        y = torch.empty((n_out, cout), dtype=torch.float32, device=x.device)
    L = _C.lib()
    ws_bytes = L.toda_spconv_fwd_workspace_bytes(x.shape[0], cin, cout, kvol, precision)
    ws = _workspace("conv", ws_bytes, x.device) if ws_bytes else None
    if precision not in _TC_PRECISIONS:
        plan = None
    with _timed(what, n_in=x.shape[0], n_out=n_out, cin=cin, cout=cout, kvol=kvol, precision=precision, rb=id(rb)):
        if plan is None and addend is None and w_bf16 is None:
            _C.check(L.toda_spconv_fwd(_p(x), _p(xb), x.shape[0], cin, _p(nbr), n_out, kvol, _p(w), cout, _p(bias), _p(y),
                                       _p(out_rows), _p(tile_masks), _p(bn_sums), precision, _p(ws), ws.numel() if ws is not None else 0,
                                       _stream()), "toda_spconv_fwd")
        else:
            pl = plan
            _C.check(L.toda_spconv_fwd_plan(_p(x), _p(xb), x.shape[0], cin, _p(nbr), n_out, kvol, _p(w), cout, _p(bias),
                                            _p(addend), _p(y), _p(out_rows), _p(tile_masks), _p(pl.lidx) if pl else None,
                                            _p(pl.rows) if pl else None, _p(pl.cnt) if pl else None, pl.ngroups if pl else 0,
                                            pl.cap if pl else 0, _p(bn_sums), _p(w_bf16), precision, _p(ws),
                                            ws.numel() if ws is not None else 0, _stream()), "toda_spconv_fwd_plan")
    return y


def conv_plan_usable(plan, cin, cout, kvol, precision):
    if plan is None or precision not in _TC_PRECISIONS or _os.environ.get("TODA_TC_FEED", "ts")[:1] in ("c",) or \
            _os.environ.get("TODA_TC_FEED", "ts")[:2] == "tm":
        return False
    cp = max(16, cin)
    return (cp in (16, 32, 64, 128) and cout in (16, 32, 64, 128) and kvol <= 27
            and plan.cap <= _C.lib().toda_tile_plan_capacity(cp))


def _conv_forward_impl(x, x_bf16, weight, bias, rb, precision, want_stats):
    x = _need(x.contiguous(), torch.float32, "features")
    weight = _need(weight.contiguous(), torch.float32, "weight")
    cout, cin = weight.shape[0], weight.shape[4]
    assert x.shape == (rb.n_in, cin), (x.shape, rb.n_in, cin)
    if x_bf16 is not None and (precision != CONV_BF16 or x_bf16.shape != x.shape or x_bf16.dtype != torch.bfloat16
                               or not x_bf16.is_contiguous()):
        x_bf16 = None
    w = _repack(weight, False, False)
    b = bias.contiguous() if bias is not None else None
    sums = None
    if want_stats and rb.n_out > 0 and _C.lib().toda_spconv_uses_tensor_cores(cin, cout, rb.kvol, precision):
        sums = torch.empty((2 * cout,), dtype=torch.float64, device=x.device)
    y = _conv_call(x, x_bf16, cin, rb.nbr_fwd, rb.n_out, rb.kvol, w, cout, b, precision, "conv_fwd", rb, sums,
                   tile_masks=rb.tile_masks, plan=rb.plan)
    return y, sums, x, weight, x_bf16


def _conv_backward_impl(dy, dyb, x, weight, xb, rb, precision, need_dx, need_dw, need_db):
    cout, cin = weight.shape[0], weight.shape[4]
    L = _C.lib()
    dx = dw = db = None
    if need_dx:
        wt = _repack(weight, True, rb.subm)
        if rb.subm:
            dx = _conv_call(dy, dyb, cout, rb.nbr_fwd, rb.n_in, rb.kvol, wt, cin, None, precision, "conv_dgrad", rb,
                            tile_masks=rb.tile_masks, plan=rb.plan)
        elif rb.dgrad_order is None:
            dx = _conv_call(dy, dyb, cout, rb.nbr_bwd, rb.n_in, rb.kvol, wt, cin, None, precision, "conv_dgrad", rb,
                            plan=rb.dgrad_plan)
        else:
            dx = _conv_call(dy, dyb, cout, rb.nbr_bwd_sorted, rb.n_in, rb.kvol, wt, cin, None, precision, "conv_dgrad",
                            rb, out_rows=rb.dgrad_order, tile_masks=rb.dgrad_tile_masks, plan=rb.dgrad_plan)
    if need_dw:
        dw = torch.empty_like(weight)
        ws_bytes = L.toda_spconv_wgrad_workspace_bytes(rb.n_in, rb.n_out, rb.kvol, cin, cout, precision)
        ws = _workspace("wgrad", ws_bytes, dy.device)
        with _timed("conv_wgrad", n_in=rb.n_in, n_out=rb.n_out, cin=cin, cout=cout, kvol=rb.kvol, precision=precision,
                    rb=id(rb)):
            _C.check(L.toda_spconv_wgrad(_p(x), _p(xb), rb.n_in, cin, _p(rb.nbr_fwd), rb.n_out, rb.kvol, _p(rb.tile_masks),
                                         _p(dy), _p(dyb), cout, _p(dw), _p(ws), ws.numel(), precision, _stream()),
                     "toda_spconv_wgrad")
    if need_db:
        db = col_sum(dy)
    return dx, dw, db


class _SparseConv(torch.autograd.Function):
    @staticmethod
    def forward(ctx, x, x_bf16, weight, bias, rb: Rulebook, precision, want_stats):
        y, sums, x, weight, x_bf16 = _conv_forward_impl(x, x_bf16, weight, bias, rb, precision, want_stats)
        ctx.save_for_backward(x, weight, x_bf16)
        ctx.set_materialize_grads(False)
        ctx.rb, ctx.precision, ctx.has_bias = rb, precision, bias is not None
        if sums is not None:
            ctx.mark_non_differentiable(sums)
        return y, sums

    @staticmethod
    def backward(ctx, dy, _dsums=None):
        if dy is None:
            return (None,) * 7
        x, weight, xb = ctx.saved_tensors
        dyb = _bf16_shadow_of(dy) if (ctx.precision == CONV_BF16 and dy.is_contiguous()) else None
        dx, dw, db = _conv_backward_impl(dy.contiguous(), dyb, x, weight, xb, ctx.rb, ctx.precision, ctx.needs_input_grad[0],
                                         ctx.needs_input_grad[2], ctx.has_bias and ctx.needs_input_grad[3])
        return dx, None, dw, db, None, None, None


def sparse_conv(x, weight, bias, rb, precision=CONV_FP32, x_bf16=None, want_stats=False):
    y, sums = _SparseConv.apply(x, x_bf16, weight, bias, rb, precision, want_stats)
    return (y, sums) if want_stats else y


def col_sum(t):
    n, c = t.shape
    out = torch.empty((c,), dtype=torch.float32, device=t.device)
    L = _C.lib()
    ws = _workspace("bn", L.toda_bn_workspace_bytes(c), t.device)
    _C.check(L.toda_col_sum(_p(t), n, c, _p(out), _p(ws), ws.numel(), _stream()), "toda_col_sum")
    return out


class ReluMaskTape:

    def __init__(self, mode):
        assert mode in ("record", "replay")
        self.mode, self.masks, self.i = mode, [], 0

    def replay(self):
        self.mode, self.i = "replay", 0
        return self


_relu_tape = None


def set_relu_mask_tape(tape):
    global _relu_tape
    _relu_tape = tape


def sync_group(bn):
    if not isinstance(bn, torch.nn.SyncBatchNorm) or not bn.training:
        return None
    if bn.momentum is None:
        raise NotImplementedError("toda_b200: SyncBatchNorm with momentum=None (cumulative moving average) is not supported; "
                                  "set a momentum (these backbones use 0.01)")
    if not (dist.is_available() and dist.is_initialized()):
        return None
    group = bn.process_group if bn.process_group is not None else dist.group.WORLD
    return group if dist.get_world_size(group) > 1 else None


def _run_phases(phases, group):
    try:
        buf = next(phases)
        while True:
            dist.all_reduce(buf, op=dist.ReduceOp.SUM, group=group)
            buf = phases.send(None)
    except StopIteration as stop:
        return stop.value


def _tape_mask(a, want_bf16):
    if _relu_tape.mode == "record":
        mask = a > 0
        _relu_tape.masks.append(mask)
    else:
        mask = _relu_tape.masks[_relu_tape.i]
        _relu_tape.i += 1
    a = a * mask
    return a, (a.to(torch.bfloat16) if want_bf16 else None), mask.to(torch.float32)


def _bn_forward_phases(y, gamma, beta, running_mean, running_var, eps, momentum, training, residual, relu, want_bf16, sums,
                       need_grad, sync=False):
    y = _need(y.contiguous(), torch.float32, "bn input")
    n, c = y.shape
    dev = y.device
    L = _C.lib()
    scale, shift, mean, rstd = torch.empty((4, c), dtype=torch.float32, device=dev).unbind(0)
    gsums = count = None
    if training:
        if sync or sums is None:
            buf = torch.empty((2 * c + 1 if sync else 2 * c,), dtype=torch.float64, device=dev)
            count = buf.data_ptr() + 16 * c if sync else None
            ws = _workspace("bn", L.toda_bn_workspace_bytes(c), dev)
            with _timed("bn_stats", n=n, c=c):
                _C.check(L.toda_bn_local_sums(_p(y), _p(sums), n, c, _p(buf), count, _p(ws), ws.numel(), _stream()),
                         "toda_bn_local_sums")
            sums = buf
        if sync:
            yield sums
            gsums = sums
    else:
        _C.check(L.toda_bn_eval_coeffs(_p(gamma), _p(beta), _p(running_mean), _p(running_var), float(eps), c, _p(scale),
                                       _p(shift), _stream()), "toda_bn_eval_coeffs")
        mean = running_mean
        rstd = torch.rsqrt(running_var + eps) if need_grad else None
    res = residual.contiguous() if residual is not None else None
    a = torch.empty_like(y)
    tape = _relu_tape is not None and relu
    ab = torch.empty(y.shape, dtype=torch.bfloat16, device=dev) if (want_bf16 and not tape) else None
    act = 0 if tape else int(relu)
    with _timed("bn_apply", n=n, c=c, residual=res is not None):
        if training:
            _C.check(L.toda_bn_apply_sums(_p(y), n, c, _p(sums), count, _p(gamma), _p(beta), float(eps), float(momentum),
                                          _p(running_mean), _p(running_var), _p(scale), _p(shift), _p(mean), _p(rstd), _p(res),
                                          act, _p(a), _p(ab), _stream()), "toda_bn_apply_sums")
        else:
            _C.check(L.toda_bn_apply(_p(y), n, c, _p(scale), _p(shift), _p(res), act, _p(a), _p(ab), _stream()), "toda_bn_apply")
    if tape:
        a, ab, mask = _tape_mask(a, want_bf16)
        return a, ab, y, mean, rstd, mask, gsums
    return a, ab, y, mean, rstd, a, gsums


def _bn_backward_phases(da, y, a, gamma, mean, rstd, training, relu, has_res, want_bf16, gsums=None, want_db=False):
    n, c = y.shape
    da = da.contiguous() if da is not None else torch.zeros_like(y)
    L = _C.lib()
    dy = torch.empty_like(y)
    dyb = torch.empty(y.shape, dtype=torch.bfloat16, device=y.device) if want_bf16 else None
    dres = torch.empty_like(y) if has_res else None
    dgamma, dbeta = torch.empty((2, c), dtype=torch.float32, device=y.device).unbind(0)
    db = torch.empty((c,), dtype=torch.float32, device=y.device) if want_db else None
    ws = _workspace("bn", L.toda_bn_workspace_bytes(c), y.device)
    if gsums is None:
        with _timed("bn_bwd", n=n, c=c, residual=has_res):
            _C.check(L.toda_bn_bwd(_p(da), _p(a), _p(y), n, c, _p(gamma), _p(mean), _p(rstd), int(relu), int(training),
                                   _p(dy), _p(dyb), _p(dres), _p(dgamma), _p(dbeta), _p(db), _p(ws), ws.numel(), _stream()),
                     "toda_bn_bwd")
        return dy, dyb, dres, dgamma, dbeta, db
    red = torch.empty((2 * c,), dtype=torch.float64, device=y.device)
    _C.check(L.toda_bn_bwd_reduce(_p(da), _p(a), _p(y), n, c, _p(mean), _p(rstd), int(relu), _p(red), _p(dgamma), _p(dbeta),
                                  _p(ws), ws.numel(), _stream()), "toda_bn_bwd_reduce")
    yield red
    _C.check(L.toda_bn_bwd_finish(_p(da), _p(a), _p(y), n, c, _p(gamma), _p(mean), _p(rstd), int(relu), 1, _p(red),
                                  gsums.data_ptr() + 16 * c, _p(dy), _p(dyb), _p(dres), _p(db), _p(ws), ws.numel(), _stream()),
             "toda_bn_bwd_finish")
    return dy, dyb, dres, dgamma, dbeta, db


class _BNAct(torch.autograd.Function):
    @staticmethod
    def forward(ctx, y, gamma, beta, running_mean, running_var, eps, momentum, training, residual, relu, want_bf16, sums, group):
        a, ab, y, mean, rstd, a_mask, gsums = _run_phases(
            _bn_forward_phases(y, gamma, beta, running_mean, running_var, eps, momentum, training, residual, relu, want_bf16, sums,
                        y.requires_grad or gamma.requires_grad, group is not None), group)
        ctx.save_for_backward(y, a_mask, gamma, mean, rstd, gsums)
        ctx.set_materialize_grads(False)
        ctx.cfg = (bool(training), bool(relu), residual is not None, bool(want_bf16))
        ctx.group = group
        if ab is not None:
            ctx.mark_non_differentiable(ab)
        return a, ab

    @staticmethod
    def backward(ctx, da, _dab=None):
        if da is None and ctx.group is None:
            return (None,) * 13
        y, a, gamma, mean, rstd, gsums = ctx.saved_tensors
        training, relu, has_res, want_bf16 = ctx.cfg
        dy, dyb, dres, dgamma, dbeta, _ = _run_phases(_bn_backward_phases(da, y, a, gamma, mean, rstd, training, relu, has_res,
                                                                          want_bf16, gsums), ctx.group)
        if dyb is not None:
            dy._toda_bf16 = (dyb, dy._version)
        return dy, dgamma, dbeta, None, None, None, None, None, dres, None, None, None, None


def _vp(t):
    return t.data_ptr() if t is not None else None


def _fused_ok(training, need_grad):
    return _prof is None and _relu_tape is None and (training or not need_grad)


def _layer_forward(x, x_bf16, weight, bias, rb, precision, gamma, beta, running_mean, running_var, eps, momentum, training,
                   residual, relu, want_bf16, need_grad=True, group=None):
    return _run_phases(_layer_forward_phases(x, x_bf16, weight, bias, rb, precision, gamma, beta, running_mean, running_var, eps,
                                             momentum, residual, relu, want_bf16, need_grad, training, group is not None), group)


def _layer_forward_phases(x, x_bf16, weight, bias, rb, precision, gamma, beta, running_mean, running_var, eps, momentum,
                          residual, relu, want_bf16, need_grad=True, training=True, sync=True):
    if not _fused_ok(training, need_grad):
        y, sums, x, weight, x_bf16 = _conv_forward_impl(x, x_bf16, weight, bias, rb, precision, bool(training))
        a, ab, y, mean, rstd, a_mask, gsums = yield from _bn_forward_phases(y, gamma, beta, running_mean, running_var, eps,
                                                                            momentum, training, residual, relu, want_bf16, sums,
                                                                            need_grad, sync)
        return a, ab, (x, x_bf16, weight, y, a_mask, gamma, mean, rstd, gsums)
    args, x, x_bf16, weight, y, a, ab, small, _keep = _layer_fwd_args(
        x, x_bf16, weight, bias, rb, precision, gamma, beta, running_mean, running_var, eps, momentum, training, residual, relu,
        want_bf16)
    cout = y.shape[1]
    L = _C.lib()
    gsums = None
    if sync:
        gsums = torch.empty((2 * cout + 1,), dtype=torch.float64, device=y.device)
        _C.check(L.toda_layer_fwd_stats(ctypes.byref(args), _p(gsums), _stream()), "toda_layer_fwd_stats")
        yield gsums
        _C.check(L.toda_layer_fwd_apply(ctypes.byref(args), _p(gsums), _stream()), "toda_layer_fwd_apply")
    else:
        _C.check(L.toda_layer_fwd(ctypes.byref(args), _stream()), "toda_layer_fwd")
    mean = small[2 * cout:3 * cout] if training else running_mean
    rstd = small[3 * cout:4 * cout] if training else None
    return a, ab, (x, x_bf16, weight, y, a, gamma, mean, rstd, gsums)


def _layer_fwd_args(x, x_bf16, weight, bias, rb, precision, gamma, beta, running_mean, running_var, eps, momentum, training,
                    residual, relu, want_bf16):
    x = _need(x.contiguous(), torch.float32, "features")
    weight = _need(weight.contiguous(), torch.float32, "weight")
    cout, cin = weight.shape[0], weight.shape[4]
    assert x.shape == (rb.n_in, cin), (x.shape, rb.n_in, cin)
    if x_bf16 is not None and (precision != CONV_BF16 or x_bf16.shape != x.shape or x_bf16.dtype != torch.bfloat16
                               or not x_bf16.is_contiguous()):
        x_bf16 = None
    L = _C.lib()
    kvol, n_out, dev = rb.kvol, rb.n_out, x.device
    tc = bool(L.toda_spconv_uses_tensor_cores(cin, cout, kvol, precision))
    if tc and precision == CONV_BF16:
        w, wb = _repack(weight, False, False, True)
    else:
        w, wb = _repack(weight, False, False), None
    y = torch.empty((n_out, cout), dtype=torch.float32, device=dev)
    a = torch.empty_like(y)
    ab = torch.empty((n_out, cout), dtype=torch.bfloat16, device=dev) if want_bf16 else None
    small = torch.empty((8 * cout,), dtype=torch.float32, device=dev)
    ws_bytes = L.toda_spconv_fwd_workspace_bytes(x.shape[0], cin, cout, kvol, precision)
    ws = _workspace("conv", ws_bytes, dev) if ws_bytes else None
    bws = _workspace("bn", L.toda_bn_workspace_bytes(cout), dev)
    res = residual.contiguous() if residual is not None else None
    b = bias.contiguous() if bias is not None else None
    pl = rb.plan if precision in _TC_PRECISIONS else None
    sp = small.data_ptr()
    args = _C.LayerFwdArgs(
        x.data_ptr(), _vp(x_bf16), x.shape[0], cin, rb.nbr_fwd.data_ptr(), n_out, kvol, w.data_ptr(), _vp(wb), cout, _vp(b),
        _vp(rb.tile_masks), _vp(pl.lidx) if pl else None, _vp(pl.rows) if pl else None, _vp(pl.cnt) if pl else None,
        pl.ngroups if pl else 0, pl.cap if pl else 0, precision, _vp(ws), ws.numel() if ws is not None else 0,
        gamma.data_ptr(), beta.data_ptr(), float(eps), float(momentum), _vp(running_mean), _vp(running_var), int(bool(training)),
        _vp(res), int(bool(relu)), y.data_ptr(), sp + 16 * cout, sp, a.data_ptr(), _vp(ab), bws.data_ptr(), bws.numel())
    return args, x, x_bf16, weight, y, a, ab, small, (w, wb, ws, bws, res, b)


def _layer_backward(da, saved, rb, precision, training, relu, has_res, has_bias, need_dx, need_dw, addend=None, group=None):
    return _run_phases(_layer_backward_phases(da, saved, rb, precision, relu, has_res, has_bias, need_dx, need_dw, addend,
                                              training), group)


def _layer_backward_phases(da, saved, rb, precision, relu, has_res, has_bias, need_dx, need_dw, addend=None, training=True):
    x, xb, weight, y, a_mask, gamma, mean, rstd, gsums = saved
    if da is None:
        da = torch.zeros_like(y)
    if not _fused_ok(training, True):
        dy, dyb, dres, dgamma, dbeta, db = yield from _bn_backward_phases(da, y, a_mask, gamma, mean, rstd, training, relu,
                                                                          has_res, precision == CONV_BF16, gsums, has_bias)
        dx, dw, _ = _conv_backward_impl(dy, dyb, x, weight, xb, rb, precision, need_dx, need_dw, False)
        if addend is not None and dx is not None:
            dx = dx + addend
        return dx, dw, db, dgamma, dbeta, dres
    args, dx, dw, dres, small, _keep = _layer_bwd_args(da, saved, rb, precision, training, relu, has_res, has_bias, need_dx,
                                                       need_dw, addend)
    cout = y.shape[1]
    L = _C.lib()
    if gsums is None:
        _C.check(L.toda_layer_bwd(ctypes.byref(args), _stream()), "toda_layer_bwd")
    else:
        red = torch.empty((2 * cout,), dtype=torch.float64, device=y.device)
        _C.check(L.toda_layer_bwd_reduce(ctypes.byref(args), _p(red), _stream()), "toda_layer_bwd_reduce")
        yield red
        _C.check(L.toda_layer_bwd_finish(ctypes.byref(args), _p(red), gsums.data_ptr() + 16 * cout, _stream()),
                 "toda_layer_bwd_finish")
    return dx, dw, (small[2 * cout:] if has_bias else None), small[:cout], small[cout:2 * cout], dres


def _layer_bwd_args(da, saved, rb, precision, training, relu, has_res, has_bias, need_dx, need_dw, addend):
    x, xb, weight, y, a_mask, gamma, mean, rstd, _ = saved
    L = _C.lib()
    da = da.contiguous()
    n_out, cout = y.shape
    cin, kvol, dev = weight.shape[4], rb.kvol, y.device
    bf16 = precision == CONV_BF16
    dy = torch.empty_like(y)
    dyb = torch.empty(y.shape, dtype=torch.bfloat16, device=dev) if bf16 else None
    dres = torch.empty_like(y) if has_res else None
    small = torch.empty((3 * cout,), dtype=torch.float32, device=dev)
    bws = _workspace("bn", L.toda_bn_workspace_bytes(cout), dev)
    dx = dw = None
    wt = wtb = None
    nbr = out_rows = masks = pl = None
    if need_dx:
        tc = bool(L.toda_spconv_uses_tensor_cores(cout, cin, kvol, precision))
        if tc and precision == CONV_BF16:
            wt, wtb = _repack(weight, True, rb.subm, True)
        else:
            wt = _repack(weight, True, rb.subm)
        if rb.subm:
            nbr, masks, pl = rb.nbr_fwd, rb.tile_masks, rb.plan
        elif rb.dgrad_order is None:
            nbr, pl = rb.nbr_bwd, rb.dgrad_plan
        else:
            nbr, out_rows, masks, pl = rb.nbr_bwd_sorted, rb.dgrad_order, rb.dgrad_tile_masks, rb.dgrad_plan
        if precision not in _TC_PRECISIONS:
            pl = None
        dx = torch.empty((rb.n_in, cin), dtype=torch.float32, device=dev)
        if addend is not None:
            addend = addend.contiguous()
    ws_bytes = L.toda_spconv_fwd_workspace_bytes(n_out, cout, cin, kvol, precision) if need_dx else 0
    ws = _workspace("conv", ws_bytes, dev) if ws_bytes else None
    wws = None
    if need_dw:
        dw = torch.empty_like(weight)
        wws = _workspace("wgrad", L.toda_spconv_wgrad_workspace_bytes(rb.n_in, n_out, kvol, cin, cout, precision), dev)
    sp = small.data_ptr()
    args = _C.LayerBwdArgs(
        da.data_ptr(), a_mask.data_ptr(), y.data_ptr(), n_out, cout, gamma.data_ptr(), _vp(mean), _vp(rstd), int(relu), int(training),
        dy.data_ptr(), _vp(dyb), _vp(dres), sp, sp + 4 * cout, bws.data_ptr(), bws.numel(),
        x.data_ptr(), _vp(xb), rb.n_in, cin, kvol,
        int(bool(need_dx)), _vp(nbr), _vp(wt), _vp(wtb), _vp(out_rows), _vp(masks),
        _vp(pl.lidx) if pl else None, _vp(pl.rows) if pl else None, _vp(pl.cnt) if pl else None, pl.ngroups if pl else 0,
        pl.cap if pl else 0, _vp(addend) if need_dx else None, _vp(dx),
        int(bool(need_dw)), rb.nbr_fwd.data_ptr(), _vp(rb.tile_masks), _vp(dw), _vp(wws), wws.numel() if wws is not None else 0,
        int(bool(has_bias)), sp + 8 * cout, precision, _vp(ws), ws.numel() if ws is not None else 0)
    return args, dx, dw, dres, small, (da, dy, dyb, addend, wt, wtb, ws, wws, bws)


class _ConvBNAct(torch.autograd.Function):

    @staticmethod
    def forward(ctx, x, x_bf16, weight, bias, rb, precision, gamma, beta, running_mean, running_var, eps, momentum, training,
                residual, relu, want_bf16, group):
        need_grad = any(ctx.needs_input_grad)
        a, ab, saved = _layer_forward(x, x_bf16, weight, bias, rb, precision, gamma, beta, running_mean, running_var, eps, momentum,
                                      training, residual, relu, want_bf16, need_grad, group)
        if need_grad:
            ctx.save_for_backward(*saved)
        ctx.set_materialize_grads(False)
        ctx.rb, ctx.precision, ctx.has_bias, ctx.group = rb, precision, bias is not None, group
        ctx.cfg = (bool(training), bool(relu), residual is not None, bool(want_bf16))
        if ab is not None:
            ctx.mark_non_differentiable(ab)
        return a, ab

    @staticmethod
    def backward(ctx, da, _dab=None):
        if da is None and ctx.group is None:
            return (None,) * 17
        training, relu, has_res, want_bf16 = ctx.cfg
        dx, dw, db, dgamma, dbeta, dres = _layer_backward(da, ctx.saved_tensors, ctx.rb, ctx.precision, training, relu, has_res,
                                                          ctx.has_bias and ctx.needs_input_grad[3], ctx.needs_input_grad[0],
                                                          ctx.needs_input_grad[2], group=ctx.group)
        return dx, None, dw, db, None, None, dgamma, dbeta, None, None, None, None, None, dres, None, None, None


class _ResBlock(torch.autograd.Function):

    @staticmethod
    def forward(ctx, x, x_bf16, w1, b1, g1, be1, rm1, rv1, w2, b2, g2, be2, rm2, rv2, rb, precision, eps, momentum, training, want_bf16,
                group1, group2):
        need_grad = any(ctx.needs_input_grad)
        h, hb, s1 = _layer_forward(x, x_bf16, w1, b1, rb, precision, g1, be1, rm1, rv1, eps, momentum, training, None, True,
                                   want_bf16, need_grad, group1)
        out, outb, s2 = _layer_forward(h, hb, w2, b2, rb, precision, g2, be2, rm2, rv2, eps, momentum, training, s1[0], True,
                                       want_bf16, need_grad, group2)
        if need_grad:
            ctx.save_for_backward(*s1, *s2)
        ctx.set_materialize_grads(False)
        ctx.rb, ctx.precision, ctx.training = rb, precision, bool(training)
        ctx.groups = (group1, group2)
        ctx.has_bias = (b1 is not None, b2 is not None)
        if outb is not None:
            ctx.mark_non_differentiable(outb)
        return out, outb

    @staticmethod
    def backward(ctx, dout, _db=None):
        if dout is None and ctx.groups == (None, None):
            return (None,) * 22
        sv = ctx.saved_tensors
        s1, s2 = sv[:9], sv[9:]
        ng = ctx.needs_input_grad
        dh, dw2, db2, dg2, dbe2, dres = _layer_backward(dout, s2, ctx.rb, ctx.precision, ctx.training, True, True,
                                                        ctx.has_bias[1] and ng[9], True, ng[8], group=ctx.groups[1])
        dx, dw1, db1, dg1, dbe1, _ = _layer_backward(dh, s1, ctx.rb, ctx.precision, ctx.training, True, False,
                                                     ctx.has_bias[0] and ng[3], ng[0], ng[2], addend=dres if ng[0] else None,
                                                     group=ctx.groups[0])
        return (dx, None, dw1, db1, dg1, dbe1, None, None, dw2, db2, dg2, dbe2, None, None, None, None, None, None, None, None,
                None, None)


def _bn_call(bn):
    group = sync_group(bn)
    training = bn.training or bn.running_mean is None
    if training and bn.running_mean is not None and bn.num_batches_tracked is not None:
        bn.num_batches_tracked += 1
    return training, group


def res_block(x, x_bf16, conv1_w, conv1_b, bn1, conv2_w, conv2_b, bn2, rb, precision, want_bf16=False):
    (training, group1), (training2, group2) = _bn_call(bn1), _bn_call(bn2)
    assert bn1.eps == bn2.eps and bn1.momentum == bn2.momentum and training == training2
    return _ResBlock.apply(x, x_bf16, conv1_w, conv1_b, bn1.weight, bn1.bias, bn1.running_mean, bn1.running_var, conv2_w, conv2_b,
                           bn2.weight, bn2.bias, bn2.running_mean, bn2.running_var, rb, precision, bn1.eps, bn1.momentum, training,
                           want_bf16, group1, group2)


def conv_bn_act(x, weight, bias, rb, precision, bn: torch.nn.BatchNorm1d, residual=None, relu=True, x_bf16=None, want_bf16=False):
    training, group = _bn_call(bn)
    return _ConvBNAct.apply(x, x_bf16, weight, bias, rb, precision, bn.weight, bn.bias, bn.running_mean, bn.running_var, bn.eps,
                            bn.momentum, training, residual, relu, want_bf16, group)


def bn_act(y, bn: torch.nn.BatchNorm1d, residual=None, relu=True, want_bf16=False, sums=None):
    training, group = _bn_call(bn)
    a, ab = _BNAct.apply(y, bn.weight, bn.bias, bn.running_mean, bn.running_var, bn.eps, bn.momentum, training, residual,
                         relu, want_bf16, sums if training else None, group)
    return (a, ab) if want_bf16 else a


class _BEVScatter(torch.autograd.Function):
    @staticmethod
    def forward(ctx, features, coords, batch, d, h, w):
        features = _need(features.contiguous(), torch.float32, "features")
        coords = _need(coords, torch.int32, "indices")
        n, c = features.shape
        out = torch.empty((batch, c * d, h, w), dtype=torch.float32, device=features.device)
        with _timed("bev_scatter_fwd", n=n, c=c, out_elems=out.numel()):
            _C.check(_C.lib().toda_bev_scatter_fwd(_p(features), _p(coords), n, c, batch, d, h, w, _p(out), _stream()),
                     "toda_bev_scatter_fwd")
        ctx.save_for_backward(coords)
        ctx.dims = (n, c, batch, d, h, w)
        return out

    @staticmethod
    def backward(ctx, dout):
        (coords,) = ctx.saved_tensors
        n, c, batch, d, h, w = ctx.dims
        dout = dout.contiguous()
        df = torch.empty((n, c), dtype=torch.float32, device=dout.device)
        with _timed("bev_scatter_bwd", n=n, c=c):
            _C.check(_C.lib().toda_bev_scatter_bwd(_p(dout), _p(coords), n, c, batch, d, h, w, _p(df), _stream()),
                     "toda_bev_scatter_bwd")
        return df, None, None, None, None, None


def bev_scatter(features, coords, batch, d, h, w):
    return _BEVScatter.apply(features, coords, batch, d, h, w)


class _GatherRows(torch.autograd.Function):
    @staticmethod
    def forward(ctx, x, rows, inverse_rows):
        x = _need(x.contiguous(), torch.float32, "features")
        n, c = rows.shape[0], x.shape[1]
        out = torch.empty((n, c), dtype=torch.float32, device=x.device)
        _C.check(_C.lib().toda_gather_rows(_p(x), _p(rows), n, c, _p(out), _stream()), "toda_gather_rows")
        ctx.save_for_backward(inverse_rows)
        return out

    @staticmethod
    def backward(ctx, dout):
        (inv,) = ctx.saved_tensors
        dout = dout.contiguous()
        n, c = inv.shape[0], dout.shape[1]
        dx = torch.empty((n, c), dtype=torch.float32, device=dout.device)
        _C.check(_C.lib().toda_gather_rows(_p(dout), _p(inv), n, c, _p(dx), _stream()), "toda_gather_rows")
        return dx, None, None


def permute_rows(x, rows, inverse_rows):
    return _GatherRows.apply(x, rows, inverse_rows)
```

Measured before the change: 420.3.

## Recompute ReLU mask from pre-BN output and saved scale/shift in BN backward

```diff
diff --git a/include/toda_b200.h b/include/toda_b200.h
--- a/include/toda_b200.h
+++ b/include/toda_b200.h
@@ -150,6 +150,7 @@
     void *wgrad_ws; size_t wgrad_ws_bytes;
     int need_db; float *db;
     int precision; void *conv_ws; size_t conv_ws_bytes;
+    const float *relu_coef;
 } toda_layer_bwd_args;
 int toda_layer_fwd(const toda_layer_fwd_args *args, void *stream);
 int toda_layer_bwd(const toda_layer_bwd_args *args, void *stream);
diff --git a/toda_b200/_C.py b/toda_b200/_C.py
--- a/toda_b200/_C.py
+++ b/toda_b200/_C.py
@@ -94,7 +94,7 @@
                 ("addend", c_vp), ("dx", c_vp),
                 ("need_dw", c_int), ("nbr_fwd", c_vp), ("fwd_masks", c_vp), ("dw", c_vp), ("wgrad_ws", c_vp), ("wgrad_ws_bytes", c_sz),
                 ("need_db", c_int), ("db", c_vp),
-                ("precision", c_int), ("conv_ws", c_vp), ("conv_ws_bytes", c_sz)]
+                ("precision", c_int), ("conv_ws", c_vp), ("conv_ws_bytes", c_sz), ("relu_coef", c_vp)]
 
 
 _lib = None
diff --git a/toda_b200/csrc/bn.cu b/toda_b200/csrc/bn.cu
--- a/toda_b200/csrc/bn.cu
+++ b/toda_b200/csrc/bn.cu
@@ -8,18 +8,26 @@
 constexpr int kPartials = 2 * kNumSMs;
 constexpr int kApplyPartials = 2048 / kThreads * kNumSMs;
 
-template <int MODE>
+__device__ __forceinline__ bool relu_open(float y, float scale, float shift) { return fmaf(y, scale, shift) > 0.f; }
+
+template <int MODE, bool YMASK = false>
 __global__ void __launch_bounds__(kThreads) col_reduce_vec_kernel(const float *__restrict__ p0, const float *__restrict__ p1,
                                                                   const float *__restrict__ p2, int n, int c,
                                                                   const float *__restrict__ mean, const float *__restrict__ rstd,
-                                                                  int relu, double *__restrict__ partial) {
+                                                                  const float *__restrict__ coef, int relu,
+                                                                  double *__restrict__ partial) {
     __shared__ double s0[kThreads * 4], s1[kThreads * 4];
     const int tpr = c >> 2;
     const int rpi = kThreads / tpr;
     const int tx = threadIdx.x % tpr, ty = threadIdx.x / tpr;
     double a0[4] = {0, 0, 0, 0}, a1[4] = {0, 0, 0, 0};
     float4 m4 = make_float4(0, 0, 0, 0), r4 = make_float4(0, 0, 0, 0);
+    float sc[4] = {0.f, 0.f, 0.f, 0.f}, sh[4] = {0.f, 0.f, 0.f, 0.f};
     if (MODE == 1) { m4 = __ldg((const float4 *)mean + tx); r4 = __ldg((const float4 *)rstd + tx); }
+    if (YMASK) {
+#pragma unroll
+        for (int q = 0; q < 4; ++q) { sc[q] = __ldg(coef + 4 * tx + q); sh[q] = __ldg(coef + c + 4 * tx + q); }
+    }
     const long long stride = (long long)gridDim.x * rpi;
     const bool active = ty < rpi;
     constexpr int U = 4;
@@ -32,7 +40,10 @@
             ok[u] = rr < n;
             size_t e = ok[u] ? (size_t)rr * tpr + tx : 0;
             v0[u] = __ldg((const float4 *)p0 + e);
-            if (MODE == 1) { v1[u] = __ldg((const float4 *)p1 + e); v2[u] = __ldg((const float4 *)p2 + e); }
+            if (MODE == 1) {
+                if (!YMASK) v1[u] = __ldg((const float4 *)p1 + e);
+                v2[u] = __ldg((const float4 *)p2 + e);
+            }
         }
 #pragma unroll
         for (int u = 0; u < U; ++u) {
@@ -42,11 +53,13 @@
 #pragma unroll
                 for (int q = 0; q < 4; ++q) { a0[q] += x[q]; a1[q] += (double)x[q] * x[q]; }
             } else if (MODE == 1) {
-                float av[4] = {v1[u].x, v1[u].y, v1[u].z, v1[u].w}, yv[4] = {v2[u].x, v2[u].y, v2[u].z, v2[u].w};
+                float yv[4] = {v2[u].x, v2[u].y, v2[u].z, v2[u].w};
                 float mm[4] = {m4.x, m4.y, m4.z, m4.w}, rs[4] = {r4.x, r4.y, r4.z, r4.w};
 #pragma unroll
                 for (int q = 0; q < 4; ++q) {
-                    float g = (relu && !(av[q] > 0.f)) ? 0.f : x[q];
+                    const bool open = YMASK ? relu_open(yv[q], sc[q], sh[q])
+                                            : (q == 0 ? v1[u].x : q == 1 ? v1[u].y : q == 2 ? v1[u].z : v1[u].w) > 0.f;
+                    float g = (relu && !open) ? 0.f : x[q];
                     float xh = (yv[q] - mm[q]) * rs[q];
                     a0[q] += g; a1[q] += (double)g * xh;
                 }
@@ -68,18 +81,20 @@
     }
 }
 
-template <int MODE>
+template <int MODE, bool YMASK = false>
 __global__ void __launch_bounds__(kThreads) col_reduce_kernel(const float *__restrict__ p0, const float *__restrict__ p1,
                                                               const float *__restrict__ p2, int n, int c,
                                                               const float *__restrict__ mean, const float *__restrict__ rstd,
-                                                              int relu, double *__restrict__ partial) {
+                                                              const float *__restrict__ coef, int relu,
+                                                              double *__restrict__ partial) {
     __shared__ double s0[kThreads], s1[kThreads];
     const int cpad = c <= 16 ? 16 : (c <= 32 ? 32 : (c <= 64 ? 64 : (c <= 128 ? 128 : 256)));
     const int rows_per_iter = kThreads / cpad;
     const int tx = threadIdx.x % cpad, ty = threadIdx.x / cpad;
     double a0 = 0.0, a1 = 0.0;
-    float m = 0.f, rs = 0.f;
+    float m = 0.f, rs = 0.f, sc = 0.f, sh = 0.f;
     if (MODE == 1 && tx < c) { m = mean[tx]; rs = rstd[tx]; }
+    if (YMASK && tx < c) { sc = coef[tx]; sh = coef[c + tx]; }
     for (long long r = (long long)blockIdx.x * rows_per_iter + ty; r < n; r += (long long)gridDim.x * rows_per_iter) {
         if (tx < c) {
             size_t e = (size_t)r * c + tx;
@@ -88,8 +103,9 @@
                 a0 += v; a1 += (double)v * v;
             } else if (MODE == 1) {
                 float g = __ldg(p0 + e);
-                if (relu && !(__ldg(p1 + e) > 0.f)) g = 0.f;
-                float xh = (__ldg(p2 + e) - m) * rs;
+                const float yv = __ldg(p2 + e);
+                if (relu && !(YMASK ? relu_open(yv, sc, sh) : __ldg(p1 + e) > 0.f)) g = 0.f;
+                float xh = (yv - m) * rs;
                 a0 += g; a1 += (double)g * xh;
             } else {
                 a0 += __ldg(p0 + e);
@@ -108,13 +124,13 @@
 
 static bool vec_channels(int c) { return c % 4 == 0 && kThreads % (c / 4) == 0; }
 
-template <int MODE>
+template <int MODE, bool YMASK = false>
 static void launch_col_reduce(const float *p0, const float *p1, const float *p2, int n, int c, const float *mean,
-                              const float *rstd, int relu, double *partial, cudaStream_t st) {
+                              const float *rstd, const float *coef, int relu, double *partial, cudaStream_t st) {
     if (vec_channels(c))
-        col_reduce_vec_kernel<MODE><<<kPartials, kThreads, 0, st>>>(p0, p1, p2, n, c, mean, rstd, relu, partial);
+        col_reduce_vec_kernel<MODE, YMASK><<<kPartials, kThreads, 0, st>>>(p0, p1, p2, n, c, mean, rstd, coef, relu, partial);
     else
-        col_reduce_kernel<MODE><<<kPartials, kThreads, 0, st>>>(p0, p1, p2, n, c, mean, rstd, relu, partial);
+        col_reduce_kernel<MODE, YMASK><<<kPartials, kThreads, 0, st>>>(p0, p1, p2, n, c, mean, rstd, coef, relu, partial);
 }
 
 template <int MAX_BLOCKS = kPartials, int ROWS = 2>
@@ -179,6 +195,10 @@
     float g = gamma ? gamma[ch] : 1.f, bt = beta ? beta[ch] : 0.f;
     scale[ch] = g * rstd;
     shift[ch] = bt - rm[ch] * g * rstd;
+}
+
+__device__ __forceinline__ long long walk_down(long long e, long long items, long long stride) {
+    return e < items ? e + (items - 1 - e) / stride * stride : -1;
 }
 
 __device__ __forceinline__ void store_bf16x4(__nv_bfloat16 *__restrict__ dst, long long e, float4 o) {
@@ -227,7 +247,7 @@
         const long long tv = total >> 2;
         const int ch = (int)((e << 2) % c);
         const float4 sc = *(const float4 *)(s_sc + ch), sh = *(const float4 *)(s_sh + ch);
-        for (; e < tv; e += stride) {
+        for (e = walk_down(e, tv, stride); e >= 0; e -= stride) {
             const float4 v = __ldg((const float4 *)y + e);
             float4 o = make_float4(fmaf(v.x, sc.x, sh.x), fmaf(v.y, sc.y, sh.y), fmaf(v.z, sc.z, sh.z), fmaf(v.w, sc.w, sh.w));
             if (residual) {
@@ -263,15 +283,21 @@
     sums[c + ch] = sx;
 }
 
-template <bool VEC>
+template <bool VEC, bool YMASK>
 __global__ void __launch_bounds__(kThreads, 5) bn_bwd_apply_kernel(const float *__restrict__ da, const float *__restrict__ a,
                                                                 const float *__restrict__ y, long long total, int c, int n,
                                                                 const double *__restrict__ count, const float *__restrict__ gamma,
                                                                 const float *__restrict__ mean, const float *__restrict__ rstd,
+                                                                const float *__restrict__ coef,
                                                                 const double *__restrict__ sums, int relu, int training,
                                                                 float *__restrict__ dy, float *__restrict__ dres,
                                                                 __nv_bfloat16 *__restrict__ dy_bf16, double *__restrict__ db_partial) {
     extern __shared__ double s_db[];
+    __shared__ float s_coef[YMASK ? 512 : 1];
+    if (YMASK) {
+        for (int i = threadIdx.x; i < 2 * c; i += blockDim.x) s_coef[i] = coef[i];
+        __syncthreads();
+    }
     double db[4] = {0.0, 0.0, 0.0, 0.0};
     if (count) n = (int)*count;
     auto sum = [&](int i) -> float { return (float)sums[i]; };
@@ -290,14 +316,21 @@
             B[q] = training ? -gm * rs * rs * sum(c + ch + q) * inv_n : 0.f;
             C[q] = training ? -A[q] * sum(ch + q) * inv_n - B[q] * mean[ch + q] : 0.f;
         }
-        for (; e < tv; e += stride) {
+        auto row = [&](long long e) {
             float4 g4 = __ldg((const float4 *)da + e);
-            float4 y4 = training ? __ldg((const float4 *)y + e) : make_float4(0.f, 0.f, 0.f, 0.f);
-            if (relu) {
+            float4 y4 = training || YMASK ? __ldg((const float4 *)y + e) : make_float4(0.f, 0.f, 0.f, 0.f);
+            if (relu && YMASK) {
+                const volatile float *sc = s_coef + ch, *sh = s_coef + c + ch;
+                g4.x = relu_open(y4.x, sc[0], sh[0]) ? g4.x : 0.f;
+                g4.y = relu_open(y4.y, sc[1], sh[1]) ? g4.y : 0.f;
+                g4.z = relu_open(y4.z, sc[2], sh[2]) ? g4.z : 0.f;
+                g4.w = relu_open(y4.w, sc[3], sh[3]) ? g4.w : 0.f;
+            } else if (relu) {
                 float4 a4 = __ldg((const float4 *)a + e);
                 g4.x = a4.x > 0.f ? g4.x : 0.f; g4.y = a4.y > 0.f ? g4.y : 0.f;
                 g4.z = a4.z > 0.f ? g4.z : 0.f; g4.w = a4.w > 0.f ? g4.w : 0.f;
             }
+            if (YMASK && !training) y4 = make_float4(0.f, 0.f, 0.f, 0.f);
             if (dres) ((float4 *)dres)[e] = g4;
             float4 o;
             o.x = fmaf(A[0], g4.x, fmaf(B[0], y4.x, C[0]));
@@ -307,12 +340,19 @@
             if (dy) ((float4 *)dy)[e] = o;
             if (dy_bf16) store_bf16x4(dy_bf16, e, o);
             if (db_partial) { db[0] += o.x; db[1] += o.y; db[2] += o.z; db[3] += o.w; }
+        };
+        e = walk_down(e, tv, stride);
+        if (YMASK) {
+#pragma unroll 2
+            for (; e >= 0; e -= stride) row(e);
+        } else {
+            for (; e >= 0; e -= stride) row(e);
         }
     } else {
         for (e = e < stride ? e : total; e < total; e += stride) {
             int ch = (int)(e % c);
             float g = __ldg(da + e);
-            if (relu && !(__ldg(a + e) > 0.f)) g = 0.f;
+            if (relu && !(YMASK ? relu_open(__ldg(y + e), coef[ch], coef[c + ch]) : __ldg(a + e) > 0.f)) g = 0.f;
             if (dres) dres[e] = g;
             float gm = gamma ? gamma[ch] : 1.f;
             float rs = rstd[ch];
@@ -396,7 +436,7 @@
     if (n > 0 && !epilogue_sums) {
         TODA_CHECK_ARG(y && workspace, "bn_local_sums: null pointer");
         if (workspace_bytes < bn_ws_bytes(c)) { toda_set_error("bn_local_sums: workspace too small"); return TODA_ERR_WORKSPACE; }
-        launch_col_reduce<0>(y, nullptr, nullptr, n, c, nullptr, nullptr, 0, (double *)workspace, st);
+        launch_col_reduce<0>(y, nullptr, nullptr, n, c, nullptr, nullptr, nullptr, 0, (double *)workspace, st);
         TODA_LAUNCH_OK();
         partial = (const double *)workspace;
     }
@@ -436,30 +476,51 @@
     return launch_bn_apply(y, n, c, k, residual, relu, a, a_bf16, (cudaStream_t)stream);
 }
 
+int bn_bwd_reduce(const float *da, const float *a, const float *y, int n, int c, const float *save_mean, const float *save_rstd,
+                  const float *relu_coef, int relu, double *local_red, float *dgamma, float *dbeta, void *workspace,
+                  size_t workspace_bytes, cudaStream_t st) {
+    TODA_CHECK_ARG(n >= 0 && c > 0 && c <= 256, "bn_bwd_reduce: unsupported sizes n=%d c=%d", n, c);
+    TODA_CHECK_ARG(save_mean && save_rstd && workspace && local_red && (n == 0 || (da && y)) && (!relu || a || relu_coef || n == 0),
+                   "bn_bwd_reduce: null pointer");
+    if (workspace_bytes < bn_ws_bytes(c)) { toda_set_error("bn_bwd_reduce: workspace too small"); return TODA_ERR_WORKSPACE; }
+    double *partial = (double *)workspace;
+    if (relu && relu_coef)
+        launch_col_reduce<1, true>(da, nullptr, y, n, c, save_mean, save_rstd, relu_coef, relu, partial, st);
+    else
+        launch_col_reduce<1>(da, a, y, n, c, save_mean, save_rstd, nullptr, relu, partial, st);
+    TODA_LAUNCH_OK();
+    bn_bwd_finalize_kernel<<<ceil_div(c * 32, 128), 128, 0, st>>>(partial, kPartials, c, dgamma, dbeta, local_red);
+    TODA_LAUNCH_OK();
+    return TODA_OK;
+}
+
 extern "C" int toda_bn_bwd_reduce(const float *da, const float *a, const float *y, int n, int c, const float *save_mean,
                                   const float *save_rstd, int relu, double *local_red, float *dgamma, float *dbeta, void *workspace,
                                   size_t workspace_bytes, void *stream) {
-    TODA_CHECK_ARG(n >= 0 && c > 0 && c <= 256, "bn_bwd_reduce: unsupported sizes n=%d c=%d", n, c);
-    TODA_CHECK_ARG(save_mean && save_rstd && workspace && local_red && (n == 0 || (da && y)) && (!relu || a || n == 0),
-                   "bn_bwd_reduce: null pointer");
-    if (workspace_bytes < bn_ws_bytes(c)) { toda_set_error("bn_bwd_reduce: workspace too small"); return TODA_ERR_WORKSPACE; }
-    cudaStream_t st = (cudaStream_t)stream;
-    double *partial = (double *)workspace;
-    launch_col_reduce<1>(da, a, y, n, c, save_mean, save_rstd, relu, partial, st);
-    TODA_LAUNCH_OK();
-    bn_bwd_finalize_kernel<<<ceil_div(c * 32, 128), 128, 0, st>>>(partial, kPartials, c, dgamma, dbeta, local_red);
-    TODA_LAUNCH_OK();
-    return TODA_OK;
-}
-
-extern "C" int toda_bn_bwd_finish(const float *da, const float *a, const float *y, int n, int c, const float *gamma,
-                                  const float *save_mean, const float *save_rstd, int relu, int training, const double *red,
-                                  const double *count, float *dy, void *dy_bf16, float *dresidual, float *dbias, void *workspace,
-                                  size_t workspace_bytes, void *stream) {
+    return bn_bwd_reduce(da, a, y, n, c, save_mean, save_rstd, nullptr, relu, local_red, dgamma, dbeta, workspace,
+                         workspace_bytes, (cudaStream_t)stream);
+}
+
+template <bool VEC>
+static void launch_bn_bwd_apply(int grid, size_t smem, cudaStream_t st, const float *da, const float *a, const float *y,
+                                long long total, int c, int n, const double *count, const float *gamma, const float *mean,
+                                const float *rstd, const float *relu_coef, const double *red, int relu, int training, float *dy,
+                                float *dres, void *dy_bf16, double *db_partial) {
+    if (relu && relu_coef)
+        bn_bwd_apply_kernel<VEC, true><<<grid, kThreads, smem, st>>>(da, nullptr, y, total, c, n, count, gamma, mean, rstd, relu_coef,
+                                                                     red, relu, training, dy, dres, (__nv_bfloat16 *)dy_bf16,
+                                                                     db_partial);
+    else
+        bn_bwd_apply_kernel<VEC, false><<<grid, kThreads, smem, st>>>(da, a, y, total, c, n, count, gamma, mean, rstd, nullptr, red,
+                                                                      relu, training, dy, dres, (__nv_bfloat16 *)dy_bf16, db_partial);
+}
+
+int bn_bwd_finish(const float *da, const float *a, const float *y, int n, int c, const float *gamma, const float *save_mean,
+                  const float *save_rstd, const float *relu_coef, int relu, int training, const double *red, const double *count,
+                  float *dy, void *dy_bf16, float *dresidual, float *dbias, void *workspace, size_t workspace_bytes, cudaStream_t st) {
     TODA_CHECK_ARG(n >= 0 && c > 0 && c <= 256, "bn_bwd_finish: unsupported sizes n=%d c=%d", n, c);
     TODA_CHECK_ARG(save_mean && save_rstd && (red || !training) && (n == 0 || (da && y && (dy || dy_bf16))) &&
-                   (!relu || a || n == 0) && (!dbias || workspace), "bn_bwd_finish: null pointer");
-    cudaStream_t st = (cudaStream_t)stream;
+                   (!relu || a || relu_coef || n == 0) && (!dbias || workspace), "bn_bwd_finish: null pointer");
     if (dbias && workspace_bytes < bn_ws_bytes(c)) { toda_set_error("bn_bwd_finish: workspace too small"); return TODA_ERR_WORKSPACE; }
     if (n == 0) {
         if (dbias) TODA_CUDA_OK(cudaMemsetAsync(dbias, 0, sizeof(float) * c, st));
@@ -470,15 +531,15 @@
     const size_t smem = dbias ? kThreads * 4 * sizeof(double) : 0;
     int grid;
     if (vec_channels(c)) {
-        grid = resident_grid<bn_bwd_apply_kernel<true>>(total / 4);
+        grid = resident_grid<bn_bwd_apply_kernel<true, false>>(total / 4);
         grid = grid < kApplyPartials ? grid : kApplyPartials;
-        bn_bwd_apply_kernel<true><<<grid, kThreads, smem, st>>>(da, a, y, total, c, n, count, gamma, save_mean, save_rstd, red, relu,
-                                                               training, dy, dresidual, (__nv_bfloat16 *)dy_bf16, db_partial);
+        launch_bn_bwd_apply<true>(grid, smem, st, da, a, y, total, c, n, count, gamma, save_mean, save_rstd, relu_coef, red, relu,
+                                  training, dy, dresidual, dy_bf16, db_partial);
     } else {
-        grid = resident_grid<bn_bwd_apply_kernel<false>>(total);
+        grid = resident_grid<bn_bwd_apply_kernel<false, false>>(total);
         grid = grid < kApplyPartials ? grid : kApplyPartials;
-        bn_bwd_apply_kernel<false><<<grid, kThreads, smem, st>>>(da, a, y, total, c, n, count, gamma, save_mean, save_rstd, red,
-                                                                relu, training, dy, dresidual, (__nv_bfloat16 *)dy_bf16, db_partial);
+        launch_bn_bwd_apply<false>(grid, smem, st, da, a, y, total, c, n, count, gamma, save_mean, save_rstd, relu_coef, red, relu,
+                                   training, dy, dresidual, dy_bf16, db_partial);
     }
     TODA_LAUNCH_OK();
     if (dbias) {
@@ -486,6 +547,14 @@
         TODA_LAUNCH_OK();
     }
     return TODA_OK;
+}
+
+extern "C" int toda_bn_bwd_finish(const float *da, const float *a, const float *y, int n, int c, const float *gamma,
+                                  const float *save_mean, const float *save_rstd, int relu, int training, const double *red,
+                                  const double *count, float *dy, void *dy_bf16, float *dresidual, float *dbias, void *workspace,
+                                  size_t workspace_bytes, void *stream) {
+    return bn_bwd_finish(da, a, y, n, c, gamma, save_mean, save_rstd, nullptr, relu, training, red, count, dy, dy_bf16, dresidual,
+                         dbias, workspace, workspace_bytes, (cudaStream_t)stream);
 }
 
 extern "C" int toda_bn_bwd(const float *da, const float *a, const float *y, int n, int c, const float *gamma,
@@ -505,7 +574,7 @@
     if (workspace_bytes < bn_ws_bytes(c)) { toda_set_error("col_sum: workspace too small"); return TODA_ERR_WORKSPACE; }
     cudaStream_t st = (cudaStream_t)stream;
     double *partial = (double *)workspace;
-    launch_col_reduce<2>(dy, nullptr, nullptr, n, c, nullptr, nullptr, 0, partial, st);
+    launch_col_reduce<2>(dy, nullptr, nullptr, n, c, nullptr, nullptr, nullptr, 0, partial, st);
     TODA_LAUNCH_OK();
     col_sum_finalize_kernel<kPartials, 2><<<ceil_div(c * 32, 128), 128, 0, st>>>(partial, kPartials, c, out);
     TODA_LAUNCH_OK();
diff --git a/toda_b200/csrc/common.cuh b/toda_b200/csrc/common.cuh
--- a/toda_b200/csrc/common.cuh
+++ b/toda_b200/csrc/common.cuh
@@ -45,6 +45,12 @@
 }
 
 double *bn_workspace_red(void *workspace, int c);
+int bn_bwd_reduce(const float *da, const float *a, const float *y, int n, int c, const float *save_mean, const float *save_rstd,
+                  const float *relu_coef, int relu, double *local_red, float *dgamma, float *dbeta, void *workspace,
+                  size_t workspace_bytes, cudaStream_t st);
+int bn_bwd_finish(const float *da, const float *a, const float *y, int n, int c, const float *gamma, const float *save_mean,
+                  const float *save_rstd, const float *relu_coef, int relu, int training, const double *red, const double *count,
+                  float *dy, void *dy_bf16, float *dresidual, float *dbias, void *workspace, size_t workspace_bytes, cudaStream_t st);
 
 struct GridIndex {
     unsigned long long *bits0;
diff --git a/toda_b200/csrc/layer.cu b/toda_b200/csrc/layer.cu
--- a/toda_b200/csrc/layer.cu
+++ b/toda_b200/csrc/layer.cu
@@ -76,16 +76,18 @@
 }
 
 static int layer_bwd_reduce(const toda_layer_bwd_args *p, double *red, void *stream) {
-    return toda_bn_bwd_reduce(p->da, p->a_mask, p->y, p->n_out, p->cout, p->mean, p->rstd, p->relu, red, p->dgamma, p->dbeta,
-                              p->bn_ws, p->bn_ws_bytes, stream);
+    TODA_CHECK_ARG(!p->relu_coef || !p->dres, "layer_bwd: relu_coef is only valid for a layer without a residual");
+    return bn_bwd_reduce(p->da, p->a_mask, p->y, p->n_out, p->cout, p->mean, p->rstd, p->relu_coef, p->relu, red, p->dgamma,
+                         p->dbeta, p->bn_ws, p->bn_ws_bytes, (cudaStream_t)stream);
 }
 
 static int layer_bwd_finish(const toda_layer_bwd_args *p, const double *red, const double *count, void *stream) {
     const int c = p->cout, n = p->n_out;
     if (n == 0) return layer_bwd_empty(p, false, (cudaStream_t)stream);
-    int rc = toda_bn_bwd_finish(p->da, p->a_mask, p->y, n, c, p->gamma, p->mean, p->rstd, p->relu, p->training, red, count,
-                                layer_bwd_reads_dy_f32(p) ? p->dy : nullptr, p->dy_bf16, p->dres, p->need_db ? p->db : nullptr,
-                                p->bn_ws, p->bn_ws_bytes, stream);
+    TODA_CHECK_ARG(!p->relu_coef || !p->dres, "layer_bwd: relu_coef is only valid for a layer without a residual");
+    int rc = bn_bwd_finish(p->da, p->a_mask, p->y, n, c, p->gamma, p->mean, p->rstd, p->relu_coef, p->relu, p->training, red, count,
+                           layer_bwd_reads_dy_f32(p) ? p->dy : nullptr, p->dy_bf16, p->dres, p->need_db ? p->db : nullptr,
+                           p->bn_ws, p->bn_ws_bytes, (cudaStream_t)stream);
     return rc ? rc : layer_bwd_conv(p, stream);
 }
 
diff --git a/toda_b200/ops.py b/toda_b200/ops.py
--- a/toda_b200/ops.py
+++ b/toda_b200/ops.py
@@ -812,7 +812,7 @@
         a, ab, y, mean, rstd, a_mask, gsums = yield from _bn_forward_phases(y, gamma, beta, running_mean, running_var, eps,
                                                                             momentum, training, residual, relu, want_bf16, sums,
                                                                             need_grad, sync)
-        return a, ab, (x, x_bf16, weight, y, a_mask, gamma, mean, rstd, gsums)
+        return a, ab, (x, x_bf16, weight, y, a_mask, gamma, mean, rstd, gsums, None)
     args, x, x_bf16, weight, y, a, ab, small, _keep = _layer_fwd_args(
         x, x_bf16, weight, bias, rb, precision, gamma, beta, running_mean, running_var, eps, momentum, training, residual, relu,
         want_bf16)
@@ -828,7 +828,8 @@
         _C.check(L.toda_layer_fwd(ctypes.byref(args), _stream()), "toda_layer_fwd")
     mean = small[2 * cout:3 * cout] if training else running_mean
     rstd = small[3 * cout:4 * cout] if training else None
-    return a, ab, (x, x_bf16, weight, y, a, gamma, mean, rstd, gsums)
+    coef = small[:2 * cout] if (relu and residual is None) else None
+    return a, ab, (x, x_bf16, weight, y, a, gamma, mean, rstd, gsums, coef)
 
 
 def _layer_fwd_args(x, x_bf16, weight, bias, rb, precision, gamma, beta, running_mean, running_var, eps, momentum, training,
@@ -873,7 +874,7 @@
 
 
 def _layer_backward_phases(da, saved, rb, precision, relu, has_res, has_bias, need_dx, need_dw, addend=None, training=True):
-    x, xb, weight, y, a_mask, gamma, mean, rstd, gsums = saved
+    x, xb, weight, y, a_mask, gamma, mean, rstd, gsums, coef = saved
     if da is None:
         da = torch.zeros_like(y)
     if not _fused_ok(training, True):
@@ -899,7 +900,7 @@
 
 
 def _layer_bwd_args(da, saved, rb, precision, training, relu, has_res, has_bias, need_dx, need_dw, addend):
-    x, xb, weight, y, a_mask, gamma, mean, rstd, _ = saved
+    x, xb, weight, y, a_mask, gamma, mean, rstd, _, coef = saved
     L = _C.lib()
     da = da.contiguous()
     n_out, cout = y.shape
@@ -938,14 +939,15 @@
         wws = _workspace("wgrad", L.toda_spconv_wgrad_workspace_bytes(rb.n_in, n_out, kvol, cin, cout, precision), dev)
     sp = small.data_ptr()
     args = _C.LayerBwdArgs(
-        da.data_ptr(), a_mask.data_ptr(), y.data_ptr(), n_out, cout, gamma.data_ptr(), _vp(mean), _vp(rstd), int(relu), int(training),
+        da.data_ptr(), _vp(a_mask), y.data_ptr(), n_out, cout, gamma.data_ptr(), _vp(mean), _vp(rstd), int(relu), int(training),
         dy.data_ptr(), _vp(dyb), _vp(dres), sp, sp + 4 * cout, bws.data_ptr(), bws.numel(),
         x.data_ptr(), _vp(xb), rb.n_in, cin, kvol,
         int(bool(need_dx)), _vp(nbr), _vp(wt), _vp(wtb), _vp(out_rows), _vp(masks),
         _vp(pl.lidx) if pl else None, _vp(pl.rows) if pl else None, _vp(pl.cnt) if pl else None, pl.ngroups if pl else 0,
         pl.cap if pl else 0, _vp(addend) if need_dx else None, _vp(dx),
         int(bool(need_dw)), rb.nbr_fwd.data_ptr(), _vp(rb.tile_masks), _vp(dw), _vp(wws), wws.numel() if wws is not None else 0,
-        int(bool(has_bias)), sp + 8 * cout, precision, _vp(ws), ws.numel() if ws is not None else 0)
+        int(bool(has_bias)), sp + 8 * cout, precision, _vp(ws), ws.numel() if ws is not None else 0,
+        _vp(coef) if relu else None)
     return args, dx, dw, dres, small, (da, dy, dyb, addend, wt, wtb, ws, wws, bws)
 
 
@@ -1002,7 +1004,7 @@
         if dout is None and ctx.groups == (None, None):
             return (None,) * 22
         sv = ctx.saved_tensors
-        s1, s2 = sv[:9], sv[9:]
+        s1, s2 = sv[:10], sv[10:]
         ng = ctx.needs_input_grad
         dh, dw2, db2, dg2, dbe2, dres = _layer_backward(dout, s2, ctx.rb, ctx.precision, ctx.training, True, True,
                                                         ctx.has_bias[1] and ng[9], True, ng[8], group=ctx.groups[1])
```

Measured after the change: 431.4, median of 6. +2.6%, better.
